# ax-le/nn-fac

Measured on AMD Instinct MI355X. Metric: HALS NMF outer iterations/s (100000x2000 rank-50 row blocks per second), higher is better.
Workload: dtype f32; 1 GPU; NMF hals beta=2, 100000x2000 rank 50 per GPU (configs[1] of BASELINE.json), deterministic (alpha=inf, delta=0.01, maxiter=100); rows_total=100000, cols=2000, rank=50, rows_per_rank=100000, parallelism=single GPU, cost_evaluation=streaming kernel (nnf_frob_resid_f32)

## Files before the change

### nn_fac_amd/csrc/k_hals.hip

```cpp
#include "k_hals_common.h"
#include <cstdlib>

__global__ void nnf_hals_prep_kernel(const float* __restrict__ UtU, int64_t ldg, int r, int RP, float* __restrict__ Gp,
                                     float* __restrict__ dinv, float* __restrict__ Gs, unsigned* counter, double* status) {
    const int RS = 32 * ((RP + 31) / 32);
    const int a = blockIdx.x;
    const float da = (a < r) ? UtU[(int64_t)a * ldg + a] : 0.f;
    const float dia = (da != 0.f) ? (float)(1.0 / (double)da) : 0.f;
    int odd = 0;
    for (int b = threadIdx.x; b < RS; b += blockDim.x) {
        const float g = (a < r && b < r) ? UtU[(int64_t)a * ldg + b] : 0.f;
        odd |= (fabsf(g) < __builtin_inff()) ? 0 : 1;
        Gp[a * RS + b] = g;
        if (Gs) Gs[a * RS + b] = g * dia;
    }
    if (Gs) {
        const int row_odd = __syncthreads_or(odd);
        if (threadIdx.x == 0 && RP < RS) Gs[a * RS + RS - 1] = row_odd ? __builtin_nanf("") : 0.f;
    }
    if (blockIdx.x != 0) return;
    for (int k = threadIdx.x; k < RP; k += blockDim.x) {
        const float d = (k < r) ? UtU[(int64_t)k * ldg + k] : 0.f;
        dinv[2 * k] = (d != 0.f) ? (float)(1.0 / (double)d) : 0.f;
        dinv[2 * k + 1] = (d != 0.f) ? 1.f : 0.f;
    }
    {
        int dead = 0;
        for (int i = threadIdx.x; i < r; i += blockDim.x) dead |= (UtU[(int64_t)i * ldg + i] == 0.f) ? 1 : 0;
        const int any_dead = __syncthreads_or(dead);
        if (threadIdx.x == 0) dinv[2 * RP] = any_dead ? 0.f : 1.f;
    }
    if (threadIdx.x == 0) {
        *counter = 0u;
        if (status) hals_status_defaults(status);
    }
}

template <int MODE, bool GCOL, bool BIG = GCOL>
__global__ __launch_bounds__(128) void nnf_hals_generic_kernel(const float* __restrict__ UtM, int64_t ldm,
                                                               const float* __restrict__ Gp, const float* __restrict__ dinv,
                                                               int RP, float* __restrict__ V, int64_t ldv, int r,
                                                               int64_t ncols, int max_sweeps, double delta, float sp,
                                                               unsigned flags, hals_sync sy, double* __restrict__ status,
                                                               double* __restrict__ sweep_partials, int sweep0,
                                                               float* __restrict__ snapshots, int64_t snap_stride, int snap_first) {
    constexpr int LPC = (BIG && !GCOL) ? 4 : 1;
    constexpr int CW = 128 / LPC;
    extern __shared__ __attribute__((aligned(16))) char smem[];
    float* vl = reinterpret_cast<float*>(smem);
    double* red = reinterpret_cast<double*>(smem + (GCOL ? (size_t)0 : (size_t)r * CW * 4) + 16);
    __shared__ unsigned lds_flag;
    const int nblocks = gridDim.x;
    const int q = threadIdx.x % LPC;
    const int64_t gcolumn = (int64_t)blockIdx.x * CW + threadIdx.x / LPC;
    const bool rowsync = (flags & (NNF_HALS_NORMALIZE | NNF_HALS_NONZERO)) != 0;
    const bool active = gcolumn < ncols;
    const bool owner = active && q == 0;
    unsigned epoch = 0;
    double eps0 = 0.0, eps = 1.0;
    int done = 0, err = 0;
    bool ok = true;
    if (MODE == 0 && sweep0 > 0 && !hals_take_over(status, sweep0, delta, eps0, eps)) return;
    const int64_t col0 = active ? gcolumn : 0;
    float* mycol = GCOL ? V + col0 : vl + threadIdx.x / LPC;
    const int64_t cs = GCOL ? ldv : CW;
    if constexpr (!GCOL) {
        for (int k = q; k < r; k += LPC) mycol[k * CW] = active ? V[(int64_t)k * ldv + col0] : 0.f;
        if constexpr (LPC > 1) __builtin_amdgcn_fence(__ATOMIC_SEQ_CST, "wavefront");
    }
    for (int s = 1; s <= max_sweeps && ok; ++s) {
        double nd = 0.0;
        for (int k = 0; k < r; ++k) {
            const float di = dinv[2 * k];
            if (di != 0.f) {
                float dot = 0.f;
                if constexpr (BIG) {
                    const float* gk = Gp + (size_t)k * RP;
                    float d[8] = {0.f, 0.f, 0.f, 0.f, 0.f, 0.f, 0.f, 0.f};
                    int i = q;
                    for (; i + 7 * LPC < r; i += 8 * LPC) {
                        float gv[8], vv[8];
#pragma unroll
                        for (int u = 0; u < 8; ++u) { gv[u] = gk[i + u * LPC]; vv[u] = mycol[(int64_t)(i + u * LPC) * cs]; }
#pragma unroll
                        for (int u = 0; u < 8; ++u) d[u] = fmaf(gv[u], vv[u], d[u]);
                    }
                    for (int u = 0; i < r; i += LPC, ++u) d[u & 7] = fmaf(gk[i], mycol[(int64_t)i * cs], d[u & 7]);
                    dot = ((d[0] + d[1]) + (d[2] + d[3])) + ((d[4] + d[5]) + (d[6] + d[7]));
                    if constexpr (LPC > 1) {
                        dot += __shfl_xor(dot, 1, 64);
                        dot += __shfl_xor(dot, 2, 64);
                    }
                } else
                for (int i = 0; i < r; ++i) dot = fmaf(Gp[k * RP + i], mycol[i * cs], dot);
                const float vk = mycol[k * cs];
                const float x = (UtM[(int64_t)k * ldm + col0] - dot - sp) * di;
                float step = !(x < -vk) ? x : -vk;
                if (!active) step = 0.f;
                if constexpr (LPC > 1) {
                    __builtin_amdgcn_fence(__ATOMIC_SEQ_CST, "wavefront");
                    if (q == 0) mycol[k * cs] = vk + step;
                    __builtin_amdgcn_fence(__ATOMIC_SEQ_CST, "wavefront");
                    if (q == 0) nd += (double)step * (double)step;
                } else {
                    if (!GCOL || active) mycol[k * cs] = vk + step;
                    nd += (double)step * (double)step;
                }
            } else if (flags & NNF_HALS_NONZERO) {
                err = 2;
            }
            if (rowsync) {
                const float vk = mycol[k * cs];
                double vmax = 0.0;
                if (flags & NNF_HALS_NONZERO) {
                    for (int i = q; i < r; i += LPC) vmax = hals_nanmax(vmax, (double)mycol[i * cs]);
                    if constexpr (LPC > 1) {
                        vmax = hals_nanmax(vmax, __shfl_xor(vmax, 1, 64));
                        vmax = hals_nanmax(vmax, __shfl_xor(vmax, 2, 64));
                    }
                }
                double mine[3] = {owner ? (double)vk * (double)vk : 0.0, (owner && vk != 0.f) ? 1.0 : 0.0,
                                  active ? vmax : -1.0e300};
                double tot[3];
                const double b0 = nnf_block_sum_f64(mine[0], red);
                const double b1 = nnf_block_sum_f64(mine[1], red);
                double bm = mine[2];
                for (int o = 32; o > 0; o >>= 1) bm = hals_nanmax(bm, __shfl_down(bm, o, 64));
                if ((threadIdx.x & 63) == 0) red[threadIdx.x >> 6] = bm;
                __syncthreads();
                bm = hals_nanmax(red[0], red[1]);
                __syncthreads();
                double pub[3] = {b0, b1, bm};
                if (threadIdx.x != 0) { pub[0] = 0; pub[1] = 0; }
                ok = grid_exchange<3>(sy, ++epoch, nblocks, pub, tot, red, &lds_flag);
                if (!ok) break;
                if ((flags & NNF_HALS_NONZERO) && di != 0.f && tot[1] == 0.0 && owner)
                    mycol[k * cs] = (float)(1e-16 * tot[2]);
                if constexpr (LPC > 1) __builtin_amdgcn_fence(__ATOMIC_SEQ_CST, "wavefront");
                if (flags & NNF_HALS_NORMALIZE) {
                    double nsq = tot[0];
                    if ((flags & NNF_HALS_NONZERO) && di != 0.f && tot[1] == 0.0) {
                        const double f = 1e-16 * tot[2];
                        nsq = f * f * (double)ncols;
                    }
                    if (owner) {
                        if (nsq != 0.0) mycol[k * cs] = (float)((double)mycol[k * cs] / sqrt(nsq));
                        else mycol[k * cs] = (float)(1.0 / sqrt((double)ncols));
                    }
                    if constexpr (LPC > 1) __builtin_amdgcn_fence(__ATOMIC_SEQ_CST, "wavefront");
                }
            }
        }
        if (!ok) break;
        done = s;
        const double bs = nnf_block_sum_f64(nd, red);
        if (MODE == 1) {
            if (threadIdx.x == 0) sweep_partials[(size_t)(s - 1) * nblocks + blockIdx.x] = bs;
            if (snapshots != nullptr && s > snap_first && active) {
                float* sn = snapshots + (int64_t)(s - 1 - snap_first) * snap_stride + col0;
                for (int k = q; k < r; k += LPC) sn[(int64_t)k * ncols] = mycol[k * cs];
            }
        } else {
            double mine[1] = {bs}, tot[1];
            ok = grid_exchange<1>(sy, ++epoch, nblocks, mine, tot, red, &lds_flag);
            if (!ok) break;
            if (!hals_note_sum(tot[0], s, sweep0, delta, eps0, eps, done)) break;
        }
    }
    if (!GCOL && active)
        for (int k = q; k < r; k += LPC) V[(int64_t)k * ldv + col0] = mycol[k * CW];
    if (blockIdx.x == 0 && threadIdx.x == 0 && status) {
        hals_status_finish(status, MODE == 0 && max_sweeps >= 1, sweep0, done, eps, eps0, !ok);
        if (ok && err) status[NNF_HALS_ST_ERR] = (double)err;
    }
}

__global__ void nnf_hals_hadamard_kernel(const float* __restrict__ A, const float* __restrict__ B, int64_t ld, int r,
                                        float* __restrict__ out) {
    const int e = blockIdx.x * 256 + threadIdx.x;
    if (e < r * r) out[e] = A[(int64_t)(e / r) * ld + (e % r)] * B[(int64_t)(e / r) * ld + (e % r)];
}

__global__ __launch_bounds__(256) void nnf_hals_sum_sweeps_kernel(const double* __restrict__ partials, int nblocks,
                                                                  double* __restrict__ out) {
    __shared__ double red[4];
    const double* p = partials + (size_t)blockIdx.x * nblocks;
    double s = 0.0;
    for (int b = threadIdx.x; b < nblocks; b += 256) s += p[b];
    const double t = nnf_block_sum_f64(s, red);
    if (threadIdx.x == 0) out[blockIdx.x] = t;
}

struct hals_request {
    int mode;
    const float* UtM; int64_t ldm;
    const float* UtU; const float* UtU2; int64_t ldg;
    float* V; int64_t ldv;
    const float* Vsrc; int64_t ldvs;
    int r; int64_t ncols;
    int nsweeps, sweep0;
    double delta; float sparsity; unsigned flags;
    double* status; double* nodelta;
    float* snapshots; int64_t snap_stride; int snap_first;
    const float* resid_in; float* resid_out;
    hals_shape shape(char force) const {
        return {mode, r, ncols, ldm, ldv, ldvs, nsweeps, sweep0, flags, UtU2 != nullptr, Vsrc != V, snapshots != nullptr, force};
    }
};

static char hals_force() {
    const char* fenv = getenv("NNF_HALS_FORCE");
    return fenv ? fenv[0] : 0;
}

typedef decltype(&nnf_hals_generic_kernel<0, false>) hals_generic_fn;
static hals_generic_fn generic_kernel(int mode, hals_layout l) {
    static const hals_generic_fn k[2][3] = {
        {nnf_hals_generic_kernel<0, false, false>, nnf_hals_generic_kernel<0, false, true>, nnf_hals_generic_kernel<0, true, true>},
        {nnf_hals_generic_kernel<1, false, false>, nnf_hals_generic_kernel<1, false, true>, nnf_hals_generic_kernel<1, true, true>}};
    return k[mode][l - HL_GENERIC_LDS];
}
static int generic_per_cu(int mode, hals_layout l, int r, size_t lds, int cap) {
    static int cached[2][3][HALS_GENERIC_LDS_MAX / 128 + 1];
    static size_t lds_set[2][3];
    const hals_generic_fn k = generic_kernel(mode, l);
    int& c = cached[mode][l - HL_GENERIC_LDS][l == HL_GENERIC_GCOL ? 0 : r];
    if (c == 0) {
        if (l != HL_GENERIC_GCOL && lds > lds_set[mode][l - HL_GENERIC_LDS]) {
            (void)hipFuncSetAttribute(reinterpret_cast<const void*>(k), hipFuncAttributeMaxDynamicSharedMemorySize, (int)lds);
            lds_set[mode][l - HL_GENERIC_LDS] = lds;
        }
        int nb = 0;
        c = hals_per_cu(hipOccupancyMaxActiveBlocksPerMultiprocessor(&nb, k, 128, lds), nb, cap) + 1;
    }
    return c - 1;
}
static const hals_occupancy hals_device_occupancy = {nnf_hals_wave_per_cu, nnf_hals_quad_per_cu, nnf_hals_fast_per_cu,
                                                     nnf_hals_mfma_per_cu, generic_per_cu};

static int hals_entry(nnf_ctx* ctx, hals_request q, hipStream_t st) {
    if (!ctx || !q.UtM || !q.UtU || !q.V || q.r < 1 || q.ncols < 1 || q.ldm < q.ncols || q.ldv < q.ncols || q.ldg < q.r || q.nsweeps < 0)
        return NNF_ERR_ARG;
    if (q.mode == 0 && !q.status) return NNF_ERR_ARG;
    if (q.mode == 1 && !q.nodelta && q.nsweeps > 0) return NNF_ERR_ARG;
    if (q.nsweeps > NNF_HALS_MAX_SWEEPS) return NNF_ERR_UNSUPPORTED;
    if (q.flags & ~(NNF_HALS_SPARSITY | NNF_HALS_NORMALIZE | NNF_HALS_NONZERO)) return NNF_ERR_ARG;
    if (q.Vsrc == nullptr || q.Vsrc == q.V) { q.Vsrc = q.V; q.ldvs = q.ldv; }
    const hals_shape shape = q.shape(hals_force());
    const hals_plan p = hals_make_plan(ctx->num_cus, hals_device_occupancy, shape);
    if (getenv("NNF_HALS_DEBUG")) hals_report(stderr, shape, p);
    if (p.err != NNF_OK) return p.err;

    const bool sweeps = q.nsweeps > 0;
    const int RS = 32 * ((p.RP + 31) / 32);
    nnf_ws_cursor cur(ctx);
    float* Gm = p.mfma_floats ? (float*)cur.take(p.mfma_floats * 4) : nullptr;
    float* Gp = (float*)cur.take(p.gram_floats * 4);
    float* dinv = Gp ? Gp + (size_t)p.RP * RS : nullptr;
    unsigned* counter = (unsigned*)cur.take(256);
    double* slots = (double*)cur.take((size_t)2 * NNF_HALS_MAX_BLOCKS * 4 * 8);
    double* sslots = (q.mode == 0) ? (double*)ctx->xch : slots;
    if (q.mode == 0 && (size_t)(q.nsweeps + 2) * NNF_HALS_MAX_BLOCKS * 16 > ctx->xch_bytes) return NNF_ERR_WORKSPACE;
    const int pslots = p.nblocks > NNF_HALS_MAX_BLOCKS ? p.nblocks : NNF_HALS_MAX_BLOCKS;
    double* partials = q.mode == 1 ? (double*)cur.take((size_t)(sweeps ? q.nsweeps : 1) * pslots * 8) : nullptr;
    float* Gh = p.hadamard ? (float*)cur.take((size_t)q.r * q.r * 4) : nullptr;
    float* snap = p.snap_floats && sweeps ? (float*)cur.take(p.snap_floats * 4) : nullptr;
    if ((p.mfma_floats && !Gm) || !Gp || !counter || !slots || (q.mode == 1 && !partials) || (p.hadamard && !Gh) ||
        (p.snap_floats && sweeps && !snap))
        return NNF_ERR_WORKSPACE;

    if (p.hadamard) {
        hipLaunchKernelGGL(nnf_hals_hadamard_kernel, dim3((q.r * q.r + 255) / 256), dim3(256), 0, st, q.UtU, q.UtU2, q.ldg, q.r, Gh);
        NNF_CHECK_LAUNCH();
        q.UtU = Gh, q.ldg = q.r, q.UtU2 = nullptr;
    }
    const bool native = p.layout == HL_WAVE || p.layout == HL_QUAD;
    auto copy_start_values = [&]() {
        const hipError_t e = hipMemcpy2DAsync(q.V, (size_t)q.ldv * 4, q.Vsrc, (size_t)q.ldvs * 4, (size_t)q.ncols * 4, (size_t)q.r,
                                              hipMemcpyDeviceToDevice, st);
        q.Vsrc = q.V, q.ldvs = q.ldv;
        return e == hipSuccess ? NNF_OK : NNF_ERR_LAUNCH;
    };
    if (p.copy && !native && copy_start_values() != NNF_OK) return NNF_ERR_LAUNCH;
    double* const status0 = (q.mode == 0 && q.sweep0 == 0) ? q.status : nullptr;
    int rc = NNF_OK;
    if (p.prep) {
        if (p.layout == HL_WAVE) rc = nnf_hals_wave_prep(q.UtU, q.UtU2, q.ldg, q.r, Gp, counter, q.status, st);
        else if (p.layout == HL_QUAD) rc = nnf_hals_quad_prep(q.UtU, q.UtU2, q.ldg, q.r, Gp, counter, status0, st);
        else {
            hipLaunchKernelGGL(nnf_hals_prep_kernel, dim3(p.RP), dim3(128), 0, st, q.UtU, q.ldg, q.r, p.RP, Gp, dinv,
                               p.gs ? Gp + hals_gs_off(p.RP) : (float*)nullptr, counter, status0);
            NNF_CHECK_LAUNCH();
        }
        if (rc != NNF_OK) return rc;
    }
    if (p.copy && native && copy_start_values() != NNF_OK) return NNF_ERR_LAUNCH;
    if (!sweeps) return NNF_OK;

    ctx->hals_epoch = (ctx->hals_epoch + 1u) & HALS_EPOCH_MASK;
    if (ctx->hals_epoch == 0u) {
        if (hipMemsetAsync(ctx->xch, 0, ctx->xch_bytes, st) != hipSuccess) return NNF_ERR_LAUNCH;
        ctx->hals_epoch = 1u;
    }
    const hals_sync sy{counter, slots, sslots, ctx->hals_epoch};
    const float sp = (q.flags & NNF_HALS_SPARSITY) ? q.sparsity : 0.f;
    hals_args a{q.UtM, q.ldm, Gp, dinv, p.gs ? Gp + hals_gs_off(p.RP) : nullptr, q.V, q.ldv, q.r, q.ncols, q.nsweeps,
                q.delta, sp, q.mode, sy, q.status, partials, q.snapshots, q.snap_stride, q.sweep0, q.Vsrc, q.ldvs};
    a.snap_first = q.snap_first, a.resid_in = q.resid_in, a.resid_out = q.resid_out;
    const bool probed = p.layout < HL_GENERIC_LDS;
    if (probed) nnf_probe(ctx, NNF_PROBE_HALS, 0, st);
    switch (p.layout) {
        case HL_WAVE:
            a.Gp = q.UtU, a.Gs = q.UtU2, a.dinv = nullptr;
            rc = nnf_hals_wave_launch(p.cpw, p.nw, a, q.ldg, snap, p.nblocks, st);
            break;
        case HL_QUAD: rc = nnf_hals_quad_launch(p.ch, a, Gp, p.nblocks, st); break;
        case HL_MFMA: rc = nnf_hals_mfma_launch(p.RP, q.UtU, q.ldg, Gm, a, p.nblocks, st); break;
        case HL_LANE_RES:
        case HL_LANE_STREAM: rc = nnf_hals_fast_launch(p.RP, p.layout == HL_LANE_RES, a, p.nblocks, st); break;
        default:
            hipLaunchKernelGGL(generic_kernel(q.mode, p.layout), dim3(p.nblocks), dim3(128), p.lds, st, q.UtM, q.ldm, Gp, dinv, RS, q.V,
                               q.ldv, q.r, q.ncols, q.nsweeps, q.delta, sp, q.flags, sy, q.status, partials, q.sweep0, q.snapshots,
                               q.snap_stride, q.snap_first);
            if (hipGetLastError() != hipSuccess) rc = NNF_ERR_LAUNCH;
    }
    if (rc != NNF_OK) return rc;
    if (probed) nnf_probe(ctx, NNF_PROBE_HALS, 1, st);
    if (q.mode == 1) {
        hipLaunchKernelGGL(nnf_hals_sum_sweeps_kernel, dim3(q.nsweeps), dim3(256), 0, st, partials, p.nblocks, q.nodelta);
        NNF_CHECK_LAUNCH();
    }
    return NNF_OK;
}

extern "C" int nnf_hals_solve_f32(nnf_ctx* ctx, const float* UtM, int64_t ldm, const float* UtU, int64_t ldg, float* V,
                                  int64_t ldv, int r, int64_t ncols, int max_sweeps, double delta, float sparsity,
                                  unsigned flags, double* status_f64, void* stream) {
    return hals_entry(ctx, {0, UtM, ldm, UtU, nullptr, ldg, V, ldv, nullptr, 0, r, ncols, max_sweeps, 0, delta, sparsity, flags, status_f64},
                      (hipStream_t)stream);
}

extern "C" int nnf_hals_sweeps_f32(nnf_ctx* ctx, const float* UtM, int64_t ldm, const float* UtU, int64_t ldg, float* V,
                                   int64_t ldv, int r, int64_t ncols, int nsweeps, float sparsity, unsigned flags,
                                   double* nodelta_f64, float* snapshots, int64_t snap_stride, void* stream) {
    return nnf_hals_sweeps_ex_f32(ctx, UtM, ldm, UtU, ldg, V, ldv, r, ncols, nsweeps, 0, sparsity, flags, nodelta_f64, snapshots,
                                  snap_stride, 0, nullptr, nullptr, stream);
}

extern "C" int nnf_hals_sweeps_ex_f32(nnf_ctx* ctx, const float* UtM, int64_t ldm, const float* UtU, int64_t ldg, float* V,
                                      int64_t ldv, int r, int64_t ncols, int nsweeps, int sweeps_done, float sparsity,
                                      unsigned flags, double* nodelta_f64, float* snapshots, int64_t snap_stride, int snap_first,
                                      const float* resid_in, float* resid_out, void* stream) {
    if (sweeps_done < 0 || snap_first < 0 || (snapshots && snap_first >= nsweeps && nsweeps > 0)) return NNF_ERR_ARG;
    if (snapshots && ((flags & (NNF_HALS_NORMALIZE | NNF_HALS_NONZERO)) || snap_stride < (int64_t)r * ncols)) return NNF_ERR_ARG;
    return hals_entry(ctx, {1, UtM, ldm, UtU, nullptr, ldg, V, ldv, nullptr, 0, r, ncols, nsweeps, sweeps_done, 0.0, sparsity, flags, nullptr,
                            nodelta_f64, snapshots, snap_stride, snap_first, resid_in, resid_out}, (hipStream_t)stream);
}

extern "C" int nnf_hals_resid_floats(nnf_ctx* ctx, int r, int64_t ncols, int64_t* floats_out) {
    if (!ctx || r < 1 || ncols < 1 || !floats_out) return NNF_ERR_ARG;
    const hals_shape blind = {1, r, ncols, ncols, ncols, ncols, 1, 0, 0u, false, false, false, hals_force()};
    const hals_plan p = hals_make_plan(ctx->num_cus, hals_device_occupancy, blind);
    *floats_out = (p.err == NNF_OK && p.layout == HL_MFMA) ? (int64_t)nnf_hals_mfma_resid_floats(p.RP, ncols) : 0;
    return NNF_OK;
}

extern "C" int nnf_hals_solve_continue_f32(nnf_ctx* ctx, const float* UtM, int64_t ldm, const float* UtU, int64_t ldg,
                                           float* V, int64_t ldv, int r, int64_t ncols, int sweeps_done, int max_sweeps,
                                           double delta, float sparsity, unsigned flags, double* status_f64, void* stream) {
    if (sweeps_done < 1 || max_sweeps < 1) return NNF_ERR_ARG;
    return hals_entry(ctx, {0, UtM, ldm, UtU, nullptr, ldg, V, ldv, nullptr, 0, r, ncols, max_sweeps, sweeps_done, delta, sparsity, flags,
                            status_f64}, (hipStream_t)stream);
}

__global__ __launch_bounds__(256) void nnf_hals_stop_restore_kernel(const double* __restrict__ sums, int nsweeps, int head,
                                                                   int budget, double delta, float* __restrict__ V, int64_t ldv,
                                                                   int r, int64_t ncols, const float* __restrict__ snapshots,
                                                                   int64_t snap_stride, double* __restrict__ status) {
    __shared__ int s_stop;
    if (threadIdx.x == 0) {
        int stop = -1;
        const double eps0 = sums[0];
        for (int s = 0; s < nsweeps; ++s)
            if (!hals_goes_on(sums[s], delta, eps0) || s + 1 >= budget) { stop = s; break; }
        s_stop = stop;
        if (blockIdx.x == 0) {
            status[NNF_HALS_ST_EPS0] = eps0;
            if (stop < 0) {
                status[NNF_HALS_ST_EPS] = sums[nsweeps - 1];
                status[NNF_HALS_ST_CNT] = (double)(nsweeps + 1);
                status[NNF_HALS_ST_ERR] = 4.0;
            } else {
                status[NNF_HALS_ST_EPS] = sums[stop];
                status[NNF_HALS_ST_CNT] = (double)(stop + 2);
                status[NNF_HALS_ST_ERR] = (stop < head) ? 3.0 : 0.0;
            }
        }
    }
    __syncthreads();
    const int stop = s_stop;
    if (stop < head || stop >= nsweeps - 1) return;
    const float* src = snapshots + (int64_t)(stop - head) * snap_stride;
    const int64_t total = (int64_t)r * ncols;
    for (int64_t e = (int64_t)blockIdx.x * 256 + threadIdx.x; e < total; e += (int64_t)gridDim.x * 256) {
        const int64_t k = e / ncols, j = e - k * ncols;
        V[k * ldv + j] = src[k * ncols + j];
    }
}

extern "C" int nnf_hals_resident_columns(nnf_ctx* ctx, int r, int64_t* columns_out) {
    if (!ctx || r < 1 || !columns_out) return NNF_ERR_ARG;
    const int64_t columns = hals_resident_columns(ctx->num_cus, hals_device_occupancy, r);
    if (columns < 1) return NNF_ERR_LAUNCH;
    *columns_out = columns;
    return NNF_OK;
}

extern "C" int nnf_hals_stop_restore_f32(nnf_ctx* ctx, const double* sums_f64, int nsweeps, int head, int budget, double delta,
                                         float* V, int64_t ldv, int r, int64_t ncols, const float* snapshots,
                                         int64_t snap_stride, double* status_f64, void* stream) {
    if (!ctx || !sums_f64 || !V || !status_f64 || nsweeps < 1 || head < 0 || head >= nsweeps || budget < 1 || r < 1 ||
        ncols < 1 || ldv < ncols)
        return NNF_ERR_ARG;
    if (nsweeps - head > 1 && (!snapshots || snap_stride < (int64_t)r * ncols)) return NNF_ERR_ARG;
    int64_t grid = nnf_cdiv((int64_t)r * ncols, 256 * 8);
    if (grid > 2048) grid = 2048;
    if (grid < 1) grid = 1;
    hipLaunchKernelGGL(nnf_hals_stop_restore_kernel, dim3((int)grid), dim3(256), 0, (hipStream_t)stream, sums_f64, nsweeps, head,
                       budget, delta, V, ldv, r, ncols, snapshots, snap_stride, status_f64);
    NNF_CHECK_LAUNCH();
    return NNF_OK;
}

extern "C" int nnf_hals_solve_cross_f32(nnf_ctx* ctx, const float* UtM, int64_t ldm, const float* UtU_a, const float* UtU_b,
                                        int64_t ldg, const float* V_in, int64_t ldvi, float* V_out, int64_t ldvo, int r,
                                        int64_t ncols, int max_sweeps, double delta, float sparsity, unsigned flags,
                                        double* status_f64, void* stream) {
    if (!V_in || ldvi < ncols) return NNF_ERR_ARG;
    if (max_sweeps > NNF_HALS_MAX_SWEEPS) return NNF_ERR_UNSUPPORTED;
    return hals_entry(ctx, {0, UtM, ldm, UtU_a, UtU_b, ldg, V_out, ldvo, V_in, ldvi, r, ncols, max_sweeps, 0, delta, sparsity, flags,
                            status_f64}, (hipStream_t)stream);
}

__global__ __launch_bounds__(256) void nnf_hals_row_update_kernel(const float* __restrict__ UtM, int64_t ldm, const float* __restrict__ UtU,
                                                                  int64_t ldg, float* __restrict__ V, int64_t ldv, int r, int64_t ncols,
                                                                  int k, float sp, double* __restrict__ partial) {
    __shared__ double red[4];
    const float d = UtU[(int64_t)k * ldg + k];
    const float di = (d != 0.f) ? (float)(1.0 / (double)d) : 0.f;
    double nd = 0.0, nv = 0.0;
    for (int64_t col = (int64_t)blockIdx.x * 256 + threadIdx.x; col < ncols; col += (int64_t)gridDim.x * 256) {
        float vk = V[(int64_t)k * ldv + col];
        if (di != 0.f) {
            float dot = 0.f;
            for (int i = 0; i < r; ++i) dot = fmaf(UtU[(int64_t)k * ldg + i], V[(int64_t)i * ldv + col], dot);
            const float x = (UtM[(int64_t)k * ldm + col] - dot - sp) * di;
            const float step = !(x < -vk) ? x : -vk;
            vk += step;
            V[(int64_t)k * ldv + col] = vk;
            nd += (double)step * (double)step;
        }
        nv += (double)vk * (double)vk;
    }
    const double bd = nnf_block_sum_f64(nd, red), bv = nnf_block_sum_f64(nv, red);
    if (threadIdx.x == 0) {
        partial[blockIdx.x] = bd;
        partial[gridDim.x + blockIdx.x] = bv;
    }
}
__global__ __launch_bounds__(256) void nnf_hals_row_sums_kernel(const double* __restrict__ partial, int nwg, double* __restrict__ out2) {
    __shared__ double red[4];
    for (int q = 0; q < 2; ++q) {
        double s = 0.0;
        for (int e = threadIdx.x; e < nwg; e += 256) s += partial[(size_t)q * nwg + e];
        const double t = nnf_block_sum_f64(s, red);
        if (threadIdx.x == 0) out2[q] = t;
    }
}
__global__ __launch_bounds__(256) void nnf_hals_row_scale_kernel(float* __restrict__ V, int64_t ncols, const double* __restrict__ normsq,
                                                                 double fill) {
    const double nsq = normsq[0];
    for (int64_t col = (int64_t)blockIdx.x * 256 + threadIdx.x; col < ncols; col += (int64_t)gridDim.x * 256)
        V[col] = (nsq != 0.0) ? (float)((double)V[col] / sqrt(nsq)) : (float)fill;
}
extern "C" int nnf_hals_row_update_f32(nnf_ctx* ctx, const float* UtM, int64_t ldm, const float* UtU, int64_t ldg, float* V, int64_t ldv,
                                       int r, int64_t ncols, int k, float sparsity, unsigned flags, double* out2_f64, void* stream) {
    if (!ctx || !UtM || !UtU || !V || !out2_f64 || r < 1 || ncols < 1 || k < 0 || k >= r || ldm < ncols || ldv < ncols || ldg < r)
        return NNF_ERR_ARG;
    if (flags & ~NNF_HALS_SPARSITY) return NNF_ERR_ARG;
    hipStream_t st = (hipStream_t)stream;
    int64_t grid = nnf_cdiv(ncols, 256);
    if (grid > 2048) grid = 2048;
    nnf_ws_cursor cur(ctx);
    double* partial = (double*)cur.take((size_t)2 * grid * 8);
    if (!partial) return NNF_ERR_WORKSPACE;
    hipLaunchKernelGGL(nnf_hals_row_update_kernel, dim3((int)grid), dim3(256), 0, st, UtM, ldm, UtU, ldg, V, ldv, r, ncols, k,
                       (flags & NNF_HALS_SPARSITY) ? sparsity : 0.f, partial);
    NNF_CHECK_LAUNCH();
    hipLaunchKernelGGL(nnf_hals_row_sums_kernel, dim3(1), dim3(256), 0, st, partial, (int)grid, out2_f64);
    NNF_CHECK_LAUNCH();
    return NNF_OK;
}
extern "C" int nnf_hals_row_scale_f32(nnf_ctx* ctx, float* V, int64_t ldv, int64_t ncols, int k, const double* normsq_f64,
                                      int64_t ncols_total, void* stream) {
    if (!ctx || !V || !normsq_f64 || ncols < 1 || k < 0 || ldv < ncols || ncols_total < ncols) return NNF_ERR_ARG;
    int64_t grid = nnf_cdiv(ncols, 256);
    if (grid > 2048) grid = 2048;
    hipLaunchKernelGGL(nnf_hals_row_scale_kernel, dim3((int)grid), dim3(256), 0, (hipStream_t)stream, V + (int64_t)k * ldv, ncols,
                       normsq_f64, 1.0 / sqrt((double)ncols_total));
    NNF_CHECK_LAUNCH();
    return NNF_OK;
}
```

### nn_fac_amd/csrc/k_hals_common.h

```cpp
#pragma once
#include "nnf_internal.h"
#include "k_hals_plan.h"

typedef __amdgpu_buffer_rsrc_t rsrc_t;
typedef float f32x2 __attribute__((ext_vector_type(2)));

#define HALS_SPIN_LIMIT (1u << 22)


struct hals_sync {
    unsigned* counter;
    double* slots;
    double* sslots;
    unsigned epoch;
};

__device__ __forceinline__ double hals_nanmax(double x, double y) { return (y > x || y != y) ? y : x; }

template <int NV>
__device__ __forceinline__ bool grid_exchange(const hals_sync& sy, unsigned epoch, int nblocks, const double (&mine)[NV],
                                              double (&out)[NV], double* red, unsigned* lds_flag) {
    double* slot = sy.slots + ((size_t)(epoch & 1) * nblocks + blockIdx.x) * 4;
    if (threadIdx.x == 0) {
#pragma unroll
        for (int i = 0; i < NV; ++i)
            __hip_atomic_store(reinterpret_cast<unsigned long long*>(slot + i), __builtin_bit_cast(unsigned long long, mine[i]),
                               __ATOMIC_RELAXED, __HIP_MEMORY_SCOPE_AGENT);
        asm volatile("s_waitcnt vmcnt(0)" ::: "memory");
        __hip_atomic_fetch_add(sy.counter, 1u, __ATOMIC_RELAXED, __HIP_MEMORY_SCOPE_AGENT);
        const unsigned target = epoch * (unsigned)nblocks;
        unsigned spins = 0, ok = 1;
        while (__hip_atomic_load(sy.counter, __ATOMIC_RELAXED, __HIP_MEMORY_SCOPE_AGENT) < target) {
            __builtin_amdgcn_s_sleep(2);
            if (++spins > HALS_SPIN_LIMIT) { ok = 0; break; }
        }
        *lds_flag = ok;
    }
    __syncthreads();
    const bool ok = (*lds_flag != 0);
    double s[NV];
#pragma unroll
    for (int i = 0; i < NV; ++i) s[i] = (i == 2) ? -1.0e300 : 0.0;
    const double* base = sy.slots + (size_t)(epoch & 1) * nblocks * 4;
    for (int b = threadIdx.x; b < nblocks; b += blockDim.x) {
#pragma unroll
        for (int i = 0; i < NV; ++i) {
            const double x = __builtin_bit_cast(
                double, __hip_atomic_load(reinterpret_cast<const unsigned long long*>(base + (size_t)b * 4 + i),
                                          __ATOMIC_RELAXED, __HIP_MEMORY_SCOPE_AGENT));
            if (i == 2) s[i] = hals_nanmax(s[i], x); else s[i] += x;
        }
    }
    const int w = threadIdx.x >> 6, nw = (blockDim.x + 63) >> 6;
#pragma unroll
    for (int i = 0; i < NV; ++i) {
        double v = s[i];
#pragma unroll
        for (int o = 32; o > 0; o >>= 1) {
            const double y = __shfl_down(v, o, 64);
            if (i == 2) v = hals_nanmax(v, y); else v += y;
        }
        if ((threadIdx.x & 63) == 0) red[w * NV + i] = v;
    }
    __syncthreads();
#pragma unroll
    for (int i = 0; i < NV; ++i) {
        double v = red[i];
        for (int k = 1; k < nw; ++k) {
            const double y = red[k * NV + i];
            if (i == 2) v = hals_nanmax(v, y); else v += y;
        }
        out[i] = v;
    }
    __syncthreads();
    return ok;
}


constexpr unsigned HALS_TAG_STRIDE = 1024u;
constexpr unsigned HALS_EPOCH_MASK = 0xffffffffu / HALS_TAG_STRIDE;
static_assert(NNF_HALS_MAX_SWEEPS + 2 <= HALS_TAG_STRIDE, "every sweep row of a launch has a tag of its own");
static_assert((HALS_EPOCH_MASK & (HALS_EPOCH_MASK + 1u)) == 0u, "the host wraps the epoch with this mask");
typedef unsigned long long hals_word;
__device__ __forceinline__ unsigned hals_tag(const hals_sync& sy, int s) { return sy.epoch * HALS_TAG_STRIDE + (unsigned)s; }
__device__ __forceinline__ const hals_word* hals_row(const hals_sync& sy, int s, int nblocks) {
    return reinterpret_cast<const hals_word*>(sy.sslots) + (size_t)s * nblocks * 2;
}
__device__ __forceinline__ double hals_granule_value(hals_word g0, hals_word g1) {
    return __builtin_bit_cast(double, (g1 << 32) | (g0 & 0xffffffffull));
}
__device__ __forceinline__ bool hals_granule_wait(const hals_word* row, int b, unsigned tag, hals_word& g0, hals_word& g1) {
    unsigned spins = 0;
    while (!((unsigned)(g0 >> 32) == tag && (unsigned)(g1 >> 32) == tag)) {
        if (spins > 0) __builtin_amdgcn_s_sleep(1);
        if (++spins > HALS_SPIN_LIMIT) return false;
        g0 = __hip_atomic_load(row + 2 * (size_t)b, __ATOMIC_RELAXED, __HIP_MEMORY_SCOPE_AGENT);
        g1 = __hip_atomic_load(row + 2 * (size_t)b + 1, __ATOMIC_RELAXED, __HIP_MEMORY_SCOPE_AGENT);
    }
    return true;
}
__device__ __forceinline__ void hals_publish(const hals_sync& sy, int s, int nblocks, double mine, bool me = threadIdx.x == 0) {
    if (me) {
        const hals_word bits = __builtin_bit_cast(hals_word, mine);
        const hals_word tag = (hals_word)hals_tag(sy, s) << 32;
        hals_word* g = reinterpret_cast<hals_word*>(sy.sslots) + ((size_t)s * nblocks + blockIdx.x) * 2;
        __hip_atomic_store(g, tag | (bits & 0xffffffffull), __ATOMIC_RELAXED, __HIP_MEMORY_SCOPE_AGENT);
        __hip_atomic_store(g + 1, tag | (bits >> 32), __ATOMIC_RELAXED, __HIP_MEMORY_SCOPE_AGENT);
    }
}
constexpr int HALS_PF = 2;
struct hals_prefetch {
    hals_word g0[HALS_PF], g1[HALS_PF];
    int s;
};
__device__ __forceinline__ void hals_collect_issue(const hals_sync& sy, int s, int nblocks, hals_prefetch& pf) {
    const hals_word* base = hals_row(sy, s, nblocks);
    pf.s = s;
#pragma unroll
    for (int i = 0; i < HALS_PF; ++i) {
        const int b = threadIdx.x + i * blockDim.x;
        pf.g0[i] = pf.g1[i] = 0ull;
        if (b < nblocks) {
            pf.g0[i] = __hip_atomic_load(base + 2 * (size_t)b, __ATOMIC_RELAXED, __HIP_MEMORY_SCOPE_AGENT);
            pf.g1[i] = __hip_atomic_load(base + 2 * (size_t)b + 1, __ATOMIC_RELAXED, __HIP_MEMORY_SCOPE_AGENT);
        }
    }
}
__device__ __forceinline__ bool hals_collect(const hals_sync& sy, int s, int nblocks, double& total, double* red,
                                             unsigned* lds_flag, const hals_prefetch* pf = nullptr) {
    if (threadIdx.x == 0) *lds_flag = 1u;
    __syncthreads();
    const unsigned tag = hals_tag(sy, s);
    const hals_word* base = hals_row(sy, s, nblocks);
    double v = 0.0;
    int i = 0;
    for (int b = threadIdx.x; b < nblocks; b += blockDim.x, ++i) {
        hals_word g0 = 0ull, g1 = 0ull;
        if (pf != nullptr && pf->s == s) {
#pragma unroll
            for (int u = 0; u < HALS_PF; ++u)
                if (u == i) { g0 = pf->g0[u]; g1 = pf->g1[u]; }
        }
        if (!hals_granule_wait(base, b, tag, g0, g1)) *lds_flag = 0u;
        v += hals_granule_value(g0, g1);
    }
    v = nnf_wave_sum_f64(v);
    const int w = threadIdx.x >> 6, nw = (blockDim.x + 63) >> 6;
    if ((threadIdx.x & 63) == 0) red[w] = v;
    __syncthreads();
    const bool ok = (*lds_flag != 0);
    double t = red[0];
    for (int k = 1; k < nw; ++k) t += red[k];
    total = t;
    __syncthreads();
    return ok;
}

#ifndef HALS_DBG
#define HALS_DBG 0
#endif
#ifndef HALS_LATE_ISSUE
#define HALS_LATE_ISSUE 1
#endif
#ifndef HALS_MID_AT
#define HALS_MID_AT(R) ((R) - 1)
#endif
struct hals_mid_none {
    __device__ __forceinline__ void operator()() const {}
};
struct hals_mid_issue {
    unsigned long long a0, a1;
    hals_prefetch& pf;
    __device__ __forceinline__ void operator()() const {
        static_assert(HALS_PF == 2, "two granule pairs per thread");
        asm volatile("global_load_dwordx2 %0, %4, off sc1\n\tglobal_load_dwordx2 %1, %4, off offset:8 sc1\n\t"
                     "global_load_dwordx2 %2, %5, off sc1\n\tglobal_load_dwordx2 %3, %5, off offset:8 sc1"
                     : "=&v"(pf.g0[0]), "=&v"(pf.g1[0]), "=&v"(pf.g0[1]), "=&v"(pf.g1[1])
                     : "v"(a0), "v"(a1));
    }
};
__device__ __forceinline__ void hals_mid_wait(hals_prefetch& pf) {
    asm volatile("s_waitcnt vmcnt(0)" : "+v"(pf.g0[0]), "+v"(pf.g1[0]), "+v"(pf.g0[1]), "+v"(pf.g1[1]));
}

__device__ __forceinline__ bool hals_collect1(const hals_sync& sy, int s, int nblocks, double& total, double* red_p,
                                              unsigned* lds_flag, const hals_prefetch& pf) {
    const unsigned tag = hals_tag(sy, s);
    const hals_word* base = hals_row(sy, s, nblocks);
    double v = 0.0;
    int i = 0;
    for (int b = threadIdx.x; b < nblocks; b += blockDim.x, ++i) {
        hals_word g0 = 0ull, g1 = 0ull;
        if (pf.s == s) {
#pragma unroll
            for (int u = 0; u < HALS_PF; ++u)
                if (u == i) { g0 = pf.g0[u]; g1 = pf.g1[u]; }
        }
        unsigned spins = 0;
        while (!((unsigned)(g0 >> 32) == tag && (unsigned)(g1 >> 32) == tag)) {
            if (spins > 0) __builtin_amdgcn_s_sleep(1);
            if (++spins > HALS_SPIN_LIMIT) { *lds_flag = 0u; break; }
            g0 = __hip_atomic_load(base + 2 * (size_t)b, __ATOMIC_RELAXED, __HIP_MEMORY_SCOPE_AGENT);
            g1 = __hip_atomic_load(base + 2 * (size_t)b + 1, __ATOMIC_RELAXED, __HIP_MEMORY_SCOPE_AGENT);
        }
        v += hals_granule_value(g0, g1);
    }
    v = nnf_wave_sum_f64(v);
    const int w = threadIdx.x >> 6, nw = (blockDim.x + 63) >> 6;
    if ((threadIdx.x & 63) == 0) red_p[w] = v;
    __syncthreads();
    double t = red_p[0];
    for (int k = 1; k < nw; ++k) t += red_p[k];
    total = t;
    return *lds_flag != 0u;
}

__device__ __forceinline__ bool hals_collect_wave(const hals_sync& sy, int s, int nblocks, double& total,
                                                  const hals_prefetch* pf = nullptr) {
    const unsigned tag = hals_tag(sy, s);
    const hals_word* base = hals_row(sy, s, nblocks);
    double v = 0.0;
    bool late = false;
    int i = 0;
    for (int b = threadIdx.x; b < nblocks; b += 64, ++i) {
        hals_word g0 = 0ull, g1 = 0ull;
        if (pf != nullptr && pf->s == s) {
#pragma unroll
            for (int u = 0; u < HALS_PF; ++u)
                if (u == i) { g0 = pf->g0[u]; g1 = pf->g1[u]; }
        }
        if (!hals_granule_wait(base, b, tag, g0, g1)) late = true;
        v += hals_granule_value(g0, g1);
    }
    total = nnf_wave_sum_f64(v);
    return __ballot(late) == 0ull;
}

template <int NT>
__device__ __forceinline__ bool hals_sum_collect1(const hals_sync& sy, double nd, double& bs, int c, int nblocks, double& total,
                                                  double* red_bs, double* red_tot, unsigned* lds_flag,
                                                  const hals_prefetch& pf) {
    static_assert(NT == 256 && HALS_PF == 2, "two granule pairs per thread cover nblocks <= 512");
    const unsigned tag = hals_tag(sy, c);
    const hals_word* base = hals_row(sy, c, nblocks);
    hals_word g0[HALS_PF], g1[HALS_PF];
    bool want[HALS_PF], need = false;
#pragma unroll
    for (int i = 0; i < HALS_PF; ++i) {
        want[i] = (int)threadIdx.x + NT * i < nblocks;
        g0[i] = (pf.s == c) ? pf.g0[i] : 0ull;
        g1[i] = (pf.s == c) ? pf.g1[i] : 0ull;
        need = need || (want[i] && !((unsigned)(g0[i] >> 32) == tag && (unsigned)(g1[i] >> 32) == tag));
    }
    if (!(HALS_DBG & 1) && __builtin_expect(__ballot(need) != 0ull, 0)) {
#pragma unroll 1
        for (int i = 0; i < HALS_PF; ++i) {
            const int b = (int)threadIdx.x + NT * i;
            hals_word a0 = i == 0 ? g0[0] : g0[HALS_PF - 1], a1 = i == 0 ? g1[0] : g1[HALS_PF - 1];
            if (b < nblocks && !hals_granule_wait(base, b, tag, a0, a1)) *lds_flag = 0u;
            if (i == 0) { g0[0] = a0; g1[0] = a1; } else { g0[HALS_PF - 1] = a0; g1[HALS_PF - 1] = a1; }
        }
    }
    double v = 0.0;
#pragma unroll
    for (int i = 0; i < HALS_PF; ++i)
        v += want[i] ? hals_granule_value(g0[i], g1[i]) : 0.0;
    v = nnf_wave_sum_f64(v);
    nd = nnf_wave_sum_f64(nd);
    constexpr int nw = NT / 64;
    const int w = threadIdx.x >> 6;
    if ((threadIdx.x & 63) == 0) { red_bs[w] = nd; red_tot[w] = v; }
    __syncthreads();
    double t = red_tot[0], b2 = red_bs[0];
#pragma unroll
    for (int k = 1; k < nw; ++k) { t += red_tot[k]; b2 += red_bs[k]; }
    total = t;
    bs = b2;
    return *lds_flag != 0u;
}
template <int NT>
__device__ __forceinline__ double hals_block_sum1(double v, double* red_p) {
    v = nnf_wave_sum_f64(v);
    constexpr int nw = NT / 64;
    const int w = threadIdx.x >> 6;
    if ((threadIdx.x & 63) == 0) red_p[w] = v;
    __syncthreads();
    double t = red_p[0];
#pragma unroll
    for (int k = 1; k < nw; ++k) t += red_p[k];
    return t;
}

struct hals_args {
    const float* UtM; int64_t ldm;
    const float* Gp;
    const float* dinv;
    const float* Gs;
    float* V; int64_t ldv;
    int r; int64_t ncols;
    int max_sweeps; double delta; float sp;
    int mode;
    hals_sync sy;
    double* status;
    double* sweep_partials;
    float* snapshots;
    int64_t snap_stride;
    int sweep0;
    const float* Vsrc;
    int64_t ldvs;
    const float* Mimg;
    const float* Mlt;
    int rp;
    const float* resid_in;
    float* resid_out;
    int snap_first;
};

__device__ __forceinline__ bool hals_goes_on(double eps, double delta, double eps0) { return eps >= delta * eps0; }
__device__ __forceinline__ bool hals_note_sum(double tot, int c, int sweep0, double delta, double& eps0, double& eps, int& done) {
    if (c == 1 && sweep0 == 0) eps0 = tot;
    eps = tot;
    done = c;
    return hals_goes_on(eps, delta, eps0);
}
__device__ __forceinline__ bool hals_take_over(const double* status, int sweep0, double delta, double& eps0, double& eps) {
    const double pe = status[NNF_HALS_ST_EPS], pe0 = status[NNF_HALS_ST_EPS0];
    if ((int)status[NNF_HALS_ST_CNT] - 1 != sweep0 || !(pe >= delta * pe0) || status[NNF_HALS_ST_ERR] != 0.0) return false;
    eps0 = pe0;
    eps = pe;
    return true;
}

__device__ __forceinline__ void hals_status_defaults(double* st, double err = 0.0) {
    st[NNF_HALS_ST_EPS] = 1.0;
    st[NNF_HALS_ST_CNT] = 1.0;
    st[NNF_HALS_ST_EPS0] = 0.0;
    st[NNF_HALS_ST_ERR] = err;
}
__device__ __forceinline__ void hals_status_finish(double* st, bool ran, int sweep0, int done, double eps, double eps0, bool timed_out) {
    if (ran) {
        st[NNF_HALS_ST_EPS] = eps;
        st[NNF_HALS_ST_CNT] = (double)(sweep0 + done + 1);
        st[NNF_HALS_ST_EPS0] = eps0;
    }
    if (timed_out) st[NNF_HALS_ST_ERR] = 1.0;
}

static inline int hals_per_cu(hipError_t e, int nb, int cap) {
    if (e != hipSuccess || nb < 1) return 0;
    const int b = nb >= 3 ? nb - 1 : nb;
    return cap > 0 && b > cap ? cap : b;
}


int nnf_hals_fast_per_cu(int RP, bool resident);
int nnf_hals_fast_launch(int RP, bool resident, const hals_args& a, int nblocks, hipStream_t);

int nnf_hals_wave_per_cu(int r, int cpw, int nw);
int nnf_hals_wave_prep(const float* UtU, const float* UtU2, int64_t ldg, int r, float* Gw, unsigned* counter, double* status,
                       hipStream_t);
int nnf_hals_wave_launch(int cpw, int nw, const hals_args& a, int64_t ldg, float* snap, int nblocks, hipStream_t);

int nnf_hals_mfma_per_cu(int RP);
int nnf_hals_mfma_launch(int RP, const float* UtU, int64_t ldg, float* gram, hals_args a, int nblocks, hipStream_t);

int nnf_hals_quad_per_cu(int ch);
int nnf_hals_quad_prep(const float* UtU, const float* UtU2, int64_t ldg, int r, float* Gq, unsigned* counter, double* status,
                       hipStream_t);
int nnf_hals_quad_launch(int ch, hals_args a, float* Gq, int nblocks, hipStream_t);
```

### nn_fac_amd/csrc/k_hals_fast.hip

```cpp
#include "k_hals_common.h"
#include "k_parts.h"

#ifndef HALS_PART
#error "compile with -DHALS_PART=<part>"
#endif
#define NNF_PART HALS_PART

NNF_BUILD_FLAGS(NNF_CAT(k_hals_fast, HALS_PART), "HALS_LATE_ISSUE=" NNF_STR(HALS_LATE_ISSUE) " HALS_MID_AT(R)=" NNF_STR(HALS_MID_AT(R)) " HALS_DBG=" NNF_STR(HALS_DBG))

typedef float f32x16 __attribute__((ext_vector_type(16)));
typedef float f32x8 __attribute__((ext_vector_type(8)));

#define NNF_SLOAD2(d0, d1, base, off) \
    asm volatile("s_load_dwordx16 %0, %2, %3\n\ts_load_dwordx16 %1, %2, %4" : "=&s"(d0), "=&s"(d1) : "s"(base), "i"((off) * 4), "i"((off) * 4 + 64))
#define NNF_SLOAD2D(d0, d1, dd, base, off, doff) \
    asm volatile("s_load_dwordx16 %0, %3, %4\n\ts_load_dwordx16 %1, %3, %5\n\ts_load_dword %2, %3, %6" \
                 : "=&s"(d0), "=&s"(d1), "=&s"(dd) : "s"(base), "i"((off) * 4), "i"((off) * 4 + 64), "i"((doff) * 4))
#define NNF_SWAIT2(d0, d1) asm volatile("s_waitcnt lgkmcnt(0)" : "+s"(d0), "+s"(d1))
#define NNF_SWAIT3(d0, d1, dd) asm volatile("s_waitcnt lgkmcnt(0)" : "+s"(d0), "+s"(d1), "+s"(dd))

template <int W>
struct sgbuf {
    f32x16 a, b;
    f32x8 q;
    f32x4 r;
};
template <int W, bool TIED>
__device__ __forceinline__ void sg_issue(sgbuf<W>& d, uint64_t base, int off) {
    constexpr int N16 = W / 16, N8 = (W % 16) / 8, N4 = (W % 8) / 4;
    static_assert(W % 4 == 0 && N16 <= 2, "piece decomposition");
    if constexpr (TIED) {
        if constexpr (N16 >= 1) asm volatile("s_load_dwordx16 %0, %1, %2" : "+s"(d.a) : "s"(base), "i"(off * 4));
        if constexpr (N16 >= 2) asm volatile("s_load_dwordx16 %0, %1, %2" : "+s"(d.b) : "s"(base), "i"(off * 4 + 64));
        if constexpr (N8 == 1) asm volatile("s_load_dwordx8 %0, %1, %2" : "+s"(d.q) : "s"(base), "i"(off * 4 + 64 * N16));
        if constexpr (N4 == 1) asm volatile("s_load_dwordx4 %0, %1, %2" : "+s"(d.r) : "s"(base), "i"(off * 4 + 64 * N16 + 32 * N8));
    } else {
        if constexpr (N16 >= 1) asm volatile("s_load_dwordx16 %0, %1, %2" : "=s"(d.a) : "s"(base), "i"(off * 4));
        if constexpr (N16 >= 2) asm volatile("s_load_dwordx16 %0, %1, %2" : "=s"(d.b) : "s"(base), "i"(off * 4 + 64));
        if constexpr (N8 == 1) asm volatile("s_load_dwordx8 %0, %1, %2" : "=s"(d.q) : "s"(base), "i"(off * 4 + 64 * N16));
        if constexpr (N4 == 1) asm volatile("s_load_dwordx4 %0, %1, %2" : "=s"(d.r) : "s"(base), "i"(off * 4 + 64 * N16 + 32 * N8));
    }
}
template <int W>
__device__ __forceinline__ void sg_arrived(sgbuf<W>& d) {
    constexpr int N16 = W / 16, N8 = (W % 16) / 8, N4 = (W % 8) / 4;
    if constexpr (N16 >= 1) asm volatile("" : "+s"(d.a));
    if constexpr (N16 >= 2) asm volatile("" : "+s"(d.b));
    if constexpr (N8 == 1) asm volatile("" : "+s"(d.q));
    if constexpr (N4 == 1) asm volatile("" : "+s"(d.r));
}
template <int W>
__device__ __forceinline__ f32x2 sg_pair(const sgbuf<W>& d, int p) {
    constexpr int N16 = W / 16, N8 = (W % 16) / 8;
    const int j = 2 * p;
    if (N16 >= 1 && j < 16) return f32x2{d.a[j], d.a[j + 1]};
    if (N16 >= 2 && j < 32) return f32x2{d.b[j - 16], d.b[j - 15]};
    const int j2 = j - 16 * N16;
    if (N8 == 1 && j2 < 8) return f32x2{d.q[j2], d.q[j2 + 1]};
    const int j3 = j2 - 8 * N8;
    return f32x2{d.r[j3], d.r[j3 + 1]};
}

template <int R, bool GUARD, class MID>
__device__ __forceinline__ float hals_sweep_column_xy(f32x2 (&v2)[R / 2], const float (&b)[R], const float* __restrict__ Gs,
                                                      const float* __restrict__ nzp, const MID& mid) {
    constexpr int RS = 64, P = R / 2, YW = 24, XW = (R - YW + 3) & ~3, XP = XW / 2;
    static_assert(YW == 24, "the Y issue statement below is written for x16 + x8");
    static_assert(R > 32 && R <= 64 && R % 2 == 0 && XW + YW <= RS && XW >= 8, "row split");
    const uint64_t base = (uint64_t)Gs, nzb = (uint64_t)nzp;
    sgbuf<XW> X;
    sgbuf<YW> Y[2];
    f32x2 dv[2];
    float nd = 0.f;
    sg_issue<XW, false>(X, base, 0);
    sg_issue<YW, false>(Y[0], base, XW);
    if constexpr (GUARD) asm volatile("s_load_dwordx2 %0, %1, %2" : "=s"(dv[0]) : "s"(nzb), "i"(0));
#pragma unroll
    for (int k = 0; k < R; ++k) {
        const int cur = k & 1, nxt = cur ^ 1;
        if (k == HALS_MID_AT(R)) mid();
        if constexpr (GUARD) asm volatile("s_waitcnt lgkmcnt(0)" : "+s"(dv[cur]));
        else asm volatile("s_waitcnt lgkmcnt(0)" ::: "memory");
        sg_arrived<XW>(X);
        sg_arrived<YW>(Y[cur]);
        if (k + 1 < R) {
            if constexpr (GUARD)
                asm volatile("s_load_dwordx16 %0, %3, %4\n\ts_load_dwordx8 %1, %3, %5\n\ts_load_dwordx2 %2, %6, %7"
                             : "=&s"(Y[nxt].a), "=&s"(Y[nxt].q), "=&s"(dv[nxt])
                             : "s"(base), "i"(((k + 1) * RS + XW) * 4), "i"(((k + 1) * RS + XW + 16) * 4), "s"(nzb),
                               "i"(8 * (k + 1)));
            else
                asm volatile("s_load_dwordx16 %0, %2, %3\n\ts_load_dwordx8 %1, %2, %4"
                             : "=&s"(Y[nxt].a), "=&s"(Y[nxt].q)
                             : "s"(base), "i"(((k + 1) * RS + XW) * 4), "i"(((k + 1) * RS + XW + 16) * 4));
        }
        f32x2 a0 = {0.f, 0.f}, a1 = {0.f, 0.f};
#pragma unroll
        for (int p = 0; p < XP; ++p) {
            const f32x2 g = sg_pair<XW>(X, p);
            if (p & 1) a1 = __builtin_elementwise_fma(g, v2[p], a1);
            else a0 = __builtin_elementwise_fma(g, v2[p], a0);
        }
        asm volatile("" : "+v"(a0), "+v"(a1));
        if (k + 1 < R) sg_issue<XW, true>(X, base, (k + 1) * RS);
#pragma unroll
        for (int p = XP; p < P; ++p) {
            const f32x2 g = sg_pair<YW>(Y[cur], p - XP);
            if (p & 1) a1 = __builtin_elementwise_fma(g, v2[p], a1);
            else a0 = __builtin_elementwise_fma(g, v2[p], a0);
        }
        const f32x2 a = a0 + a1;
        const float vk = v2[k / 2][k & 1];
        const float x = b[k] - (a[0] + a[1]);
        float dl;
        if constexpr (GUARD) {
            const float sel = !(x < -vk) ? x : -vk;
            asm("v_mul_legacy_f32 %0, %1, %2" : "=v"(dl) : "s"(dv[cur][1]), "v"(sel));
        } else {
            asm("v_max_f32 %0, %1, -%2" : "=v"(dl) : "v"(x), "v"(vk));
        }
        v2[k / 2][k & 1] = vk + dl;
        nd = fmaf(dl, dl, nd);
        asm volatile("" : "+v"(nd));
    }
    return nd;
}

template <int R, bool KEEPB, class MID>
__device__ __forceinline__ float hals_sweep_column(f32x2 (&v2)[R / 2], const float (&b)[KEEPB ? R : 1], rsrc_t rb, int voff,
                                                   int ldm4, const float* __restrict__ Gp, float sp, const MID& mid) {
    constexpr int NBLK = (R + 31) / 32, RS = 32 * NBLK, P = R / 2, DOFF = R * RS;
    const uint64_t base = (uint64_t)Gp;
    f32x16 buf[2][2];
    float dv[2];
    float nd = 0.f;
    constexpr int BPF = 8;
    float bring[KEEPB ? 1 : BPF];
    if constexpr (!KEEPB) {
#pragma unroll
        for (int i = 0; i < BPF; ++i)
            bring[i] = __builtin_bit_cast(float, __builtin_amdgcn_raw_buffer_load_b32(rb, voff, i * ldm4, 0));
    }
    NNF_SLOAD2D(buf[0][0], buf[0][1], dv[0], base, 0, DOFF);
#pragma unroll
    for (int k = 0; k < R; ++k) {
        if (k == HALS_MID_AT(R)) mid();
        f32x2 a0 = {0.f, 0.f}, a1 = {0.f, 0.f}, a2 = {0.f, 0.f}, a3 = {0.f, 0.f};
        float di = 0.f;
#pragma unroll
        for (int blk = 0; blk < NBLK; ++blk) {
            const int jb = k * NBLK + blk, cur = jb & 1, nxt = cur ^ 1;
            if (blk == 0) {
                NNF_SWAIT3(buf[cur][0], buf[cur][1], dv[k & 1]);
                di = dv[k & 1];
            } else {
                NNF_SWAIT2(buf[cur][0], buf[cur][1]);
            }
            if (blk + 1 < NBLK) {
                NNF_SLOAD2(buf[nxt][0], buf[nxt][1], base, k * RS + 32 * (blk + 1));
            } else if (k + 1 < R) {
                NNF_SLOAD2D(buf[nxt][0], buf[nxt][1], dv[(k + 1) & 1], base, (k + 1) * RS, DOFF + 2 * (k + 1));
            }
#pragma unroll
            for (int j = 0; j < 8; j += 2) {
                if (16 * blk + j < P)
                    a0 = __builtin_elementwise_fma(f32x2{buf[cur][0][2 * j], buf[cur][0][2 * j + 1]}, v2[16 * blk + j], a0);
                if (16 * blk + 8 + j < P)
                    a1 = __builtin_elementwise_fma(f32x2{buf[cur][1][2 * j], buf[cur][1][2 * j + 1]}, v2[16 * blk + 8 + j], a1);
                if (16 * blk + j + 1 < P)
                    a2 = __builtin_elementwise_fma(f32x2{buf[cur][0][2 * j + 2], buf[cur][0][2 * j + 3]}, v2[16 * blk + j + 1], a2);
                if (16 * blk + 8 + j + 1 < P)
                    a3 = __builtin_elementwise_fma(f32x2{buf[cur][1][2 * j + 2], buf[cur][1][2 * j + 3]}, v2[16 * blk + 8 + j + 1], a3);
            }
        }
        const f32x2 a = (a0 + a1) + (a2 + a3);
        const float dot = a[0] + a[1];
        float bk;
        if constexpr (KEEPB) {
            bk = b[k];
        } else {
            bk = bring[k % BPF];
            if (k + BPF < R)
                bring[k % BPF] = __builtin_bit_cast(float, __builtin_amdgcn_raw_buffer_load_b32(rb, voff, (k + BPF) * ldm4, 0));
        }
        const float vk = v2[k / 2][k & 1];
        const bool skip = __builtin_bit_cast(unsigned, di) == 0u;
        const float res = KEEPB ? (bk - dot) : (bk - dot - sp);
        const float x = (skip ? 0.f : res) * di;
        const float t = vk + x;
        const bool keep = !(t <= 0.f) | skip;
        const float vn = keep ? t : 0.f;
        const float step = keep ? x : -vk;
        v2[k / 2][k & 1] = vn;
        nd = fmaf(step, step, nd);
        asm volatile("" : "+v"(nd));
    }
    return nd;
}

template <int RP, bool RES>
__global__ __launch_bounds__(256, (RP > 104 ? 1 : 2)) void nnf_hals_kernel(hals_args a) {
    constexpr bool KEEPB = (RP <= 104);
    constexpr bool XY = (RP > 32 && RP <= 52);
    const bool all_live = XY && (a.dinv[2 * RP] != 0.f);
    __shared__ double red[4 * 3];
    __shared__ double red2[2][2][4];
    __shared__ unsigned lds_flag;
    if (threadIdx.x == 0) lds_flag = 1u;
    const int nblocks = gridDim.x;
    const int64_t gthreads = (int64_t)nblocks * 256;
    const int64_t gtid = (int64_t)blockIdx.x * 256 + threadIdx.x;
    const rsrc_t rv = __builtin_amdgcn_make_buffer_rsrc(a.V, 0, (int)(((int64_t)(a.r - 1) * a.ldv + a.ncols) * 4), 0x00020000);
    const rsrc_t rb = __builtin_amdgcn_make_buffer_rsrc(const_cast<float*>(a.UtM), 0,
                                                        (int)(((int64_t)(a.r - 1) * a.ldm + a.ncols) * 4), 0x00020000);
    const int ldv4 = (int)(a.ldv * 4), ldm4 = (int)(a.ldm * 4);
    const rsrc_t rvs = __builtin_amdgcn_make_buffer_rsrc(const_cast<float*>(a.Vsrc), 0,
                                                         (int)(((int64_t)(a.r - 1) * a.ldvs + a.ncols) * 4), 0x00020000);
    const int ldvs4 = (int)(a.ldvs * 4);
    f32x2 v2[RP / 2];
    float b[KEEPB ? RP : 1];
    bool plain = false;
    auto sweep = [&](int voff, const auto& mid) -> float {
        if constexpr (XY) {
            return plain ? hals_sweep_column_xy<RP, false>(v2, b, a.Gs, a.dinv, mid) : hals_sweep_column_xy<RP, true>(v2, b, a.Gs, a.dinv, mid);
        } else {
            return hals_sweep_column<RP, KEEPB>(v2, b, rb, voff, ldm4, a.Gp, a.sp, mid);
        }
    };
    auto load_col = [&](int voff) {
#pragma unroll
        for (int k = 0; k < RP; ++k) {
            v2[k / 2][k & 1] = RES ? __builtin_bit_cast(float, __builtin_amdgcn_raw_buffer_load_b32(rvs, voff, k * ldvs4, 0))
                                   : __builtin_bit_cast(float, __builtin_amdgcn_raw_buffer_load_b32(rv, voff, k * ldv4, 0));
            if constexpr (KEEPB) {
                b[k] = __builtin_bit_cast(float, __builtin_amdgcn_raw_buffer_load_b32(rb, voff, k * ldm4, 0)) - a.sp;
                if constexpr (XY) b[k] *= a.dinv[2 * k];
            }
        }
    };
    auto store_col = [&](int voff) {
#pragma unroll
        for (int k = 0; k < RP; ++k) {
            const float val = v2[k / 2][k & 1];
            __builtin_amdgcn_raw_buffer_store_b32(__builtin_bit_cast(unsigned, val), rv, voff, k * ldv4, 0);
        }
    };
    const int voff0 = gtid < a.ncols ? (int)(gtid * 4) : (int)0x7ffffff0;
    if constexpr (RES) load_col(voff0);
    if constexpr (RES && XY) {
        static_assert(!XY || RP < 64, "the scaled Gram's rows have a spare last float");
        float c = a.Gs[(threadIdx.x & 63) < RP ? (threadIdx.x & 63) * 64 + 63 : 63];
#pragma unroll
        for (int k = 0; k < RP; ++k) {
            c = fmaf(v2[k / 2][k & 1], 0.f, c);
            c = fmaf(b[k], 0.f, c);
            asm volatile("" : "+v"(c));
        }
        plain = all_live && __ballot(!(c == 0.f)) == 0ull;
    }
    constexpr bool BACKUP = RES && RP <= 64;
    constexpr bool SPEC = BACKUP;
    f32x2 vb[BACKUP ? RP / 2 : 1];

    double eps0 = 0.0, eps = 1.0;
    int done = 0;
    bool ok = true, stopped = false;
    if (a.mode == 0 && a.sweep0 > 0 && !hals_take_over(a.status, a.sweep0, a.delta, eps0, eps)) return;
    hals_prefetch pf;
    pf.s = 0;
    for (int s = 1; s <= a.max_sweeps; ++s) {
        double nd = 0.0;
        if constexpr (BACKUP) {
            if (a.mode == 0) {
#pragma unroll
                for (int k = 0; k < RP / 2; ++k) vb[k] = v2[k];
            }
        }
        if constexpr (RES) {
            float f;
            if constexpr (SPEC && (RP > 52 || !HALS_LATE_ISSUE)) {
                if (a.mode == 0 && s >= 2) hals_collect_issue(a.sy, s - 1, nblocks, pf);
                f = sweep(voff0, hals_mid_none{});
            } else if constexpr (SPEC) {
                const bool want = a.mode == 0 && s >= 2;
                const hals_word* row = hals_row(a.sy, want ? s - 1 : 0, nblocks);
                const int b0 = (int)threadIdx.x < nblocks ? (int)threadIdx.x : 0;
                const int b1 = (int)threadIdx.x + 256 < nblocks ? (int)threadIdx.x + 256 : 0;
                pf.s = want ? s - 1 : 0;
                f = sweep(voff0, hals_mid_issue{(unsigned long long)(row + 2 * (size_t)b0), (unsigned long long)(row + 2 * (size_t)b1), pf});
                hals_mid_wait(pf);
            } else {
                f = sweep(voff0, hals_mid_none{});
            }
            nd = gtid < a.ncols ? (double)f : 0.0;
        } else {
            for (int64_t col = gtid; col < a.ncols; col += gthreads) {
                const int voff = (int)(col * 4);
                load_col(voff);
                nd += (double)sweep(voff, hals_mid_none{});
                store_col(voff);
            }
        }
        double bs;
        bool merged = false;
        double tot_m = 0.0;
        if constexpr (RES && SPEC) {
            if (a.mode == 0 && s >= 2 && !(HALS_DBG & 6)) {
                ok = hals_sum_collect1<256>(a.sy, nd, bs, s - 1, nblocks, tot_m, red2[s & 1][0], red2[s & 1][1], &lds_flag, pf);
                merged = true;
            }
        }
        if (!merged) {
            if constexpr (RES) bs = hals_block_sum1<256>(nd, red2[s & 1][0]);
            else bs = nnf_block_sum_f64(nd, red);
        }
        if (a.mode == 1) {
            if (threadIdx.x == 0) a.sweep_partials[(size_t)(s - 1) * nblocks + blockIdx.x] = bs;
            if constexpr (RES) {
                if (a.snapshots != nullptr && gtid < a.ncols && s > a.snap_first) {
                    float* sp_ = a.snapshots + (size_t)(s - 1 - a.snap_first) * a.snap_stride + gtid;
#pragma unroll
                    for (int k = 0; k < RP; ++k)
                        if (k < a.r) sp_[(int64_t)k * a.ncols] = v2[k / 2][k & 1];
                }
            }
            done = s;
            continue;
        }
        if (!(HALS_DBG & 4)) hals_publish(a.sy, s, nblocks, bs);
        const int c = SPEC ? s - 1 : s;
        if (c >= 1 && !(HALS_DBG & 6)) {
            double tot;
            if (merged) tot = tot_m;
            else if constexpr (RES) ok = hals_collect1(a.sy, c, nblocks, tot, red2[s & 1][1], &lds_flag, pf);
            else ok = hals_collect(a.sy, c, nblocks, tot, red, &lds_flag, &pf);
            if (!ok) break;
            if (c == 1 && a.sweep0 == 0) eps0 = tot;
            eps = tot;
            done = c;
            if (!(eps >= a.delta * eps0) && !HALS_DBG) { stopped = true; break; }
        }
    }
    if constexpr (RES) {
        if (a.mode == 0) {
            if constexpr (BACKUP) {
                if (stopped || !ok) {
#pragma unroll
                    for (int k = 0; k < RP / 2; ++k) v2[k] = vb[k];
                }
            }
            if (a.max_sweeps >= 1) store_col(voff0);
        }
    }
    if (a.mode == 1) {
        if constexpr (RES) store_col(voff0);
    } else if (SPEC && ok && !stopped && a.max_sweeps >= 1 && !HALS_DBG) {
        double tot;
        ok = hals_collect(a.sy, a.max_sweeps, nblocks, tot, red, &lds_flag);
        if (ok) {
            if (a.max_sweeps == 1 && a.sweep0 == 0) eps0 = tot;
            eps = tot;
            done = a.max_sweeps;
        }
    }
    if (a.mode == 0 && blockIdx.x == 0 && threadIdx.x == 0)
        hals_status_finish(a.status, a.max_sweeps >= 1, a.sweep0, done, eps, eps0, !ok);
}

template <int RP>
static int fast_per_cu(bool res) {
    static int cached[2] = {-1, -1};
    int& c = cached[res ? 1 : 0];
    if (c < 0) {
        int nb = 0;
        const hipError_t e = res ? hipOccupancyMaxActiveBlocksPerMultiprocessor(&nb, nnf_hals_kernel<RP, true>, 256, 0)
                                 : hipOccupancyMaxActiveBlocksPerMultiprocessor(&nb, nnf_hals_kernel<RP, false>, 256, 0);
        c = hals_per_cu(e, nb, 3);
    }
    return c;
}

template <int RP>
static int fast_launch(bool res, const hals_args& a, int nblocks, hipStream_t st) {
    if (res) hipLaunchKernelGGL((nnf_hals_kernel<RP, true>), dim3(nblocks), dim3(256), 0, st, a);
    else hipLaunchKernelGGL((nnf_hals_kernel<RP, false>), dim3(nblocks), dim3(256), 0, st, a);
    NNF_CHECK_LAUNCH();
    return NNF_OK;
}

#define HALS_TABLE(X)                                                                                            \
    X(0, 8) X(0, 16) X(0, 24) X(0, 32) X(0, 40) X(0, 48)                                                         \
    X(1, 50) X(1, 52) X(1, 56) X(1, 64)                                                                          \
    X(2, 80) X(2, 96)                                                                                            \
    X(3, 100)                                                                                                    \
    X(4, 104)                                                                                                    \
    X(5, 112) X(5, 128)
NNF_PART_DISPATCHER(fast_mine, HALS_TABLE)

int NNF_CAT(nnf_hals_fast_per_cu_part, HALS_PART)(int RP, bool res) {
    return fast_mine(RP, 0, [&](auto rp) { return fast_per_cu<decltype(rp)::value>(res); });
}
int NNF_CAT(nnf_hals_fast_launch_part, HALS_PART)(int RP, bool res, const hals_args& a, int nblocks, hipStream_t st) {
    return fast_mine(RP, NNF_ERR_UNSUPPORTED, [&](auto rp) { return fast_launch<decltype(rp)::value>(res, a, nblocks, st); });
}

#if HALS_PART == 0
#define HALS_DECLARE(p, v)                                      \
    int NNF_PART_FN(nnf_hals_fast_per_cu_part, p)(int, bool);   \
    int NNF_PART_FN(nnf_hals_fast_launch_part, p)(int, bool, const hals_args&, int, hipStream_t);
#define HALS_PER_CU(p, v) case v: return NNF_PART_FN(nnf_hals_fast_per_cu_part, p)(RP, res);
#define HALS_LAUNCH(p, v) case v: return NNF_PART_FN(nnf_hals_fast_launch_part, p)(RP, res, a, nblocks, st);
HALS_TABLE(HALS_DECLARE)
int nnf_hals_fast_per_cu(int RP, bool res) {
    switch (RP) { HALS_TABLE(HALS_PER_CU) default: return 0; }
}
int nnf_hals_fast_launch(int RP, bool res, const hals_args& a, int nblocks, hipStream_t st) {
    switch (RP) { HALS_TABLE(HALS_LAUNCH) default: return NNF_ERR_UNSUPPORTED; }
}
#endif
```

### nn_fac_amd/csrc/k_hals_plan.h

```cpp
#pragma once
#include "k_stream_plan.h"

#define NNF_HALS_MAX_SWEEPS 1000
#define NNF_HALS_MAX_BLOCKS 2048

enum hals_layout { HL_WAVE, HL_QUAD, HL_MFMA, HL_LANE_RES, HL_LANE_STREAM, HL_GENERIC_LDS, HL_GENERIC_BIG, HL_GENERIC_GCOL };
static const char* const hals_layout_name[] = {"wave", "quad", "mfma", "lane-resident", "lane-streaming", "generic-lds",
                                               "generic-lds-big", "generic-gcol"};

struct hals_shape {
    int mode;
    int r; int64_t ncols;
    int64_t ldm, ldv, ldvs;
    int nsweeps, sweep0;
    unsigned flags;
    bool gram2;
    bool own_start;
    bool snapshots;
    char force;
};

struct hals_plan {
    int err = NNF_OK;
    hals_layout layout = HL_LANE_RES;
    int RP = 0, nblocks = 0, per_cu = 0;
    int cpw = 0, nw = 0, ch = 0;
    size_t lds = 0;
    bool hadamard = false, copy = false, prep = true;
    bool gs = false;
    size_t gram_floats = 0, mfma_floats = 0, snap_floats = 0;
};

struct hals_occupancy {
    int (*wave)(int r, int cpw, int nw);
    int (*quad)(int ch);
    int (*lane)(int RP, bool resident);
    int (*mfma)(int RP);
    int (*generic)(int mode, hals_layout layout, int r, size_t lds_bytes, int cap);
};

static inline int pick_rp(int r) {
    const int opts[] = {8, 16, 24, 32, 40, 48, 50, 52, 56, 64, 80, 96, 100, 104, 112, 128};
    for (int o : opts)
        if (r <= o) return o;
    return (r + 7) & ~7;
}

constexpr int WAVE_COMM = 4;
constexpr int WAVE_MAX_NW = 16 - WAVE_COMM;
constexpr int WAVE_SNAP = 16;
constexpr int WAVE_NP = 6;
static inline int wave_ru(int r) { return (r + 7) & ~7; }
static inline int wave_rl(int r) { return r <= 64 ? 1 : 2; }
static inline size_t nnf_hals_wave_gram_floats(int r) { return (size_t)wave_ru(r) * 64 * wave_rl(r) + 128; }
static inline size_t nnf_hals_wave_snap_floats(int r, int64_t ncols) { return (size_t)ncols * WAVE_SNAP * 64 * wave_rl(r); }
static inline int nnf_hals_wave_grid(int64_t ncols, int cpw, int* nw_out) {
    int nw = (int)nnf_cdiv(ncols, 256);
    if (nw < 1) nw = 1;
    if (nw > WAVE_MAX_NW) nw = WAVE_MAX_NW;
    *nw_out = nw;
    const int64_t need = nnf_cdiv(ncols, (int64_t)nw * cpw);
    return need > 64 * WAVE_NP ? 0 : (int)need;
}

static inline size_t nnf_hals_quad_gram_floats(int r) {
    const int ch = (r + 3) / 4, rq = 4 * ch, rs = 4 * ((ch + 3) & ~3);
    return (size_t)rq * rs + rq;
}

struct mfma_shape { int rt, rem, nkb; };
static inline bool mfma_shape_of(int RP, mfma_shape& s) {
    switch (RP) {
        case 48: s = {3, 0, 12}; return true;
        case 50: s = {3, 2, 13}; return true;
        case 52: s = {3, 4, 13}; return true;
        case 64: s = {4, 0, 16}; return true;
        case 80: s = {5, 0, 20}; return true;
        case 96: s = {6, 0, 24}; return true;
        case 100: s = {6, 4, 25}; return true;
        default: return false;
    }
}
static inline bool nnf_hals_mfma_supported(int RP) { mfma_shape s; return mfma_shape_of(RP, s); }
static inline size_t nnf_hals_mfma_gram_floats(int RP) {
    mfma_shape s;
    if (!mfma_shape_of(RP, s)) return 0;
    return (size_t)s.nkb * ((s.rt + 3) / 4) * 256 + (size_t)s.nkb * 32 + 64;
}
static inline size_t nnf_hals_mfma_resid_floats(int RP, int64_t ncols) {
    mfma_shape s;
    if (!mfma_shape_of(RP, s) || ncols < 1) return 0;
    return (size_t)nnf_cdiv(ncols, 256) * 4 * (s.rt * 4 + 1) * 256;
}

constexpr size_t HALS_GENERIC_LDS_MAX = (size_t)150 * 1024;
constexpr size_t HALS_GENERIC_SHM_FIXED = 16 + 3 * 2 * 8 + 64;

static inline int64_t hals_cap(int cus, int per_cu) {
    const int64_t c = (int64_t)per_cu * cus;
    return c < NNF_HALS_MAX_BLOCKS ? c : NNF_HALS_MAX_BLOCKS;
}
static inline bool hals_32bit(int rows, int64_t ld, int64_t ncols) {
    return (((int64_t)(rows - 1) * ld + ncols) * 4) < (int64_t)0x7fff0000;
}

static inline size_t hals_gs_off(int RP) { return ((((size_t)RP * (32 * ((RP + 31) / 32)) + 2 * RP + 1) + 15) & ~(size_t)15); }

static inline hals_plan hals_refuse(hals_plan p, int err) { p.err = err; return p; }

static inline hals_plan hals_make_plan(int cus, const hals_occupancy& occ, const hals_shape& q) {
    hals_plan p;
    const int r = q.r; const int64_t n = q.ncols;
    const bool rowsync = (q.flags & (NNF_HALS_NORMALIZE | NNF_HALS_NONZERO)) != 0;
    const bool generic = r > NNF_MAX_RANK || rowsync;
    const bool sweeps = q.nsweeps > 0;
    const char force = q.force;
    p.RP = pick_rp(r);
    const bool mfma = !generic && sweeps && force != 'l' && force != 'q' && force != 'w' && nnf_hals_mfma_supported(p.RP) &&
                      (force == 'm' || (p.RP >= 64 && n > 32768));
    const bool pin_mfma = force == 'm' && mfma;

    const bool wave_shape = !generic && q.mode == 0 && q.sweep0 == 0;
    if (wave_shape && force != 'l' && force != 'q' && !pin_mfma) {
        for (int cpw = 1; cpw <= 2; ++cpw) {
            int nw = 0;
            const int need = nnf_hals_wave_grid(n, cpw, &nw);
            if (need < 1 || need > NNF_HALS_MAX_BLOCKS) continue;
            const int pc = occ.wave(r, cpw, nw);
            if (pc < 1) break;
            if (need <= (int64_t)pc * cus) {
                p.layout = HL_WAVE, p.cpw = cpw, p.nw = nw, p.nblocks = need, p.per_cu = pc;
                p.prep = !sweeps;
                p.copy = !sweeps && q.own_start;
                p.gram_floats = nnf_hals_wave_gram_floats(r);
                p.snap_floats = nnf_hals_wave_snap_floats(r, n);
                return p;
            }
        }
    }
    if (force == 'w' && wave_shape) return hals_refuse(p, NNF_ERR_UNSUPPORTED);

    auto quad_32bit = [&](int64_t ld) { return (int64_t)(r + 16) * ld * 4 < (int64_t)0x7fff0000; };
    if (!generic && force != 'l' && !pin_mfma && (n <= 32768 || force == 'q') && quad_32bit(q.ldv > q.ldm ? q.ldv : q.ldm)) {
        const int ch = (r + 3) / 4, pc = occ.quad(ch);
        const int64_t need = nnf_cdiv(n, 16);
        if (pc > 0 && need <= hals_cap(cus, pc)) {
            p.layout = HL_QUAD, p.ch = ch, p.nblocks = (int)need, p.per_cu = pc;
            p.copy = q.own_start && (!sweeps || !quad_32bit(q.ldvs));
            p.gram_floats = nnf_hals_quad_gram_floats(r);
            return p;
        }
    }

    const int RS = 32 * ((p.RP + 31) / 32);
    p.gs = !generic && p.RP > 32 && p.RP <= 52;
    p.gram_floats = hals_gs_off(p.RP) + (p.gs ? (size_t)p.RP * RS : 0);
    p.hadamard = q.gram2;
    const int lane_pc = generic ? 0 : occ.lane(p.RP, true);
    const bool lane_fits = lane_pc > 0 && nnf_cdiv(n, 256) <= hals_cap(cus, lane_pc);
    p.copy = q.own_start && !(!generic && sweeps && lane_fits && hals_32bit(p.RP, q.ldvs, n));
    if (!sweeps) {
        p.layout = generic ? HL_GENERIC_LDS : HL_LANE_RES;
        return p;
    }

    if (generic) {
        const bool exchanges = q.mode == 0 || rowsync;
        if (r > NNF_MAX_RANK) {
            p.layout = HL_GENERIC_BIG;
            p.lds = (size_t)r * 32 * 4 + HALS_GENERIC_SHM_FIXED;
            p.per_cu = p.lds <= HALS_GENERIC_LDS_MAX ? occ.generic(q.mode, HL_GENERIC_BIG, r, p.lds, 0) : 0;
            if (p.per_cu < 1 || (exchanges && nnf_cdiv(n, 32) > hals_cap(cus, p.per_cu))) {
                p.layout = HL_GENERIC_GCOL;
                p.lds = HALS_GENERIC_SHM_FIXED;
                p.per_cu = occ.generic(q.mode, HL_GENERIC_GCOL, r, p.lds, 4);
            }
        } else {
            p.layout = HL_GENERIC_LDS;
            p.lds = (size_t)r * 128 * 4 + HALS_GENERIC_SHM_FIXED;
            p.per_cu = occ.generic(q.mode, HL_GENERIC_LDS, r, p.lds, 4);
        }
        if (p.per_cu < 1) return hals_refuse(p, NNF_ERR_LAUNCH);
        const int64_t grid = nnf_cdiv(n, p.layout == HL_GENERIC_BIG ? 32 : 128);
        if (grid > (exchanges ? hals_cap(cus, p.per_cu) : (int64_t)0x7fffffff)) return hals_refuse(p, NNF_ERR_UNSUPPORTED);
        p.nblocks = (int)grid;
        return p;
    }

    if (!hals_32bit(p.RP, q.ldv, n) || !hals_32bit(p.RP, q.ldm, n)) return hals_refuse(p, NNF_ERR_UNSUPPORTED);
    const int64_t need = nnf_cdiv(n, 256);
    if (mfma) {
        const int pc = occ.mfma(p.RP);
        if (pc > 0 && need <= hals_cap(cus, pc)) {
            p.layout = HL_MFMA, p.nblocks = (int)need, p.per_cu = pc;
            p.mfma_floats = nnf_hals_mfma_gram_floats(p.RP);
            return p;
        }
    }
    if (lane_pc < 1) return hals_refuse(p, NNF_ERR_LAUNCH);
    if (lane_fits) {
        p.layout = HL_LANE_RES, p.nblocks = (int)need, p.per_cu = lane_pc;
        return p;
    }
    if (q.snapshots) return hals_refuse(p, NNF_ERR_UNSUPPORTED);
    p.layout = HL_LANE_STREAM, p.per_cu = occ.lane(p.RP, false);
    if (p.per_cu < 1) return hals_refuse(p, NNF_ERR_LAUNCH);
    p.nblocks = (int)hals_cap(cus, p.per_cu);
    return p;
}

static inline void hals_report(FILE* f, const hals_shape& q, const hals_plan& p, const char* more = "") {
    fprintf(f, "[nnf hals] r=%d ncols=%lld mode=%d sweeps=%d sweep0=%d flags=%u -> %s grid=%d per_cu=%d cpw=%d nw=%d ch=%d "
            "RP=%d gs=%d lds=%zu hadamard=%d copy=%d prep=%d err=%d%s\n", q.r, (long long)q.ncols, q.mode, q.nsweeps, q.sweep0,
            q.flags, hals_layout_name[p.layout], p.nblocks, p.per_cu, p.cpw, p.nw, p.ch, p.RP, p.gs, p.lds, p.hadamard, p.copy,
            p.prep, p.err, more);
}

static inline int64_t hals_resident_columns(int cus, const hals_occupancy& occ, int r) {
    if (r > NNF_MAX_RANK) return hals_cap(cus, occ.generic(0, HL_GENERIC_GCOL, r, HALS_GENERIC_SHM_FIXED, 4)) * 128;
    return hals_cap(cus, occ.lane(pick_rp(r), true)) * 256;
}
```

Baseline: 1299 iterations/s.

## Add lane-resident HALS kernel with a dedicated wave for convergence reduction

Adds a new resident HALS kernel for ranks 33–52. Each 576-thread workgroup has eight compute waves that sweep 512 columns, plus one extra wave that does the grid-wide delta reduction and convergence verdict asynchronously. The compute waves go on to the next sweep without waiting for the grid exchange, and restore a saved copy of V if the verdict says to stop. This is meant to hide grid-synchronisation latency behind computation. The right-hand side moves to LDS, and the planner picks this path when the column count needs more lane blocks than there are CUs. The cost is one block per CU, one extra speculative sweep at the end, and extra register copies of V.

New measurement: 1335 iterations/s, median of 6. 1.03x the previous value.

```diff
diff --git a/nn_fac_amd/csrc/k_hals.hip b/nn_fac_amd/csrc/k_hals.hip
--- a/nn_fac_amd/csrc/k_hals.hip
+++ b/nn_fac_amd/csrc/k_hals.hip
@@ -236,7 +236,7 @@
     return c - 1;
 }
 static const hals_occupancy hals_device_occupancy = {nnf_hals_wave_per_cu, nnf_hals_quad_per_cu, nnf_hals_fast_per_cu,
-                                                     nnf_hals_mfma_per_cu, generic_per_cu};
+                                                     nnf_hals_mfma_per_cu, generic_per_cu, nnf_hals_comm_per_cu};
 
 static int hals_entry(nnf_ctx* ctx, hals_request q, hipStream_t st) {
     if (!ctx || !q.UtM || !q.UtU || !q.V || q.r < 1 || q.ncols < 1 || q.ldm < q.ncols || q.ldv < q.ncols || q.ldg < q.r || q.nsweeps < 0)
@@ -317,6 +317,8 @@
         case HL_QUAD: rc = nnf_hals_quad_launch(p.ch, a, Gp, p.nblocks, st); break;
         case HL_MFMA: rc = nnf_hals_mfma_launch(p.RP, q.UtU, q.ldg, Gm, a, p.nblocks, st); break;
         case HL_LANE_RES:
+            if (p.comm) { rc = nnf_hals_comm_launch(p.RP, a, p.nblocks, st); break; }
+            [[fallthrough]];
         case HL_LANE_STREAM: rc = nnf_hals_fast_launch(p.RP, p.layout == HL_LANE_RES, a, p.nblocks, st); break;
         default:
             hipLaunchKernelGGL(generic_kernel(q.mode, p.layout), dim3(p.nblocks), dim3(128), p.lds, st, q.UtM, q.ldm, Gp, dinv, RS, q.V,
diff --git a/nn_fac_amd/csrc/k_hals_comm.hip b/nn_fac_amd/csrc/k_hals_comm.hip
--- /dev/null
+++ b/nn_fac_amd/csrc/k_hals_comm.hip
@@ -0,0 +1,245 @@
+#include "k_hals_common.h"
+#include "k_hals_lane_sweep.h"
+
+constexpr int LC_CW = 8;
+constexpr int LC_COLS = 64 * LC_CW;
+constexpr int LC_THREADS = LC_COLS + 64;
+constexpr int LC_RING = 4;
+constexpr int LC_NP = 8;
+static_assert(LC_COLS == HALS_B_PITCH, "one row of b_lds holds the workgroup's columns");
+
+struct lane_ctl {
+    unsigned tag[LC_RING][LC_CW];
+    unsigned long long ver[LC_RING];
+    unsigned fin;
+};
+static inline size_t lc_lds_bytes(int RP) { return ((size_t)RP + 2) * LC_COLS * 4 + sizeof(lane_ctl); }
+
+#define LC_WG __HIP_MEMORY_SCOPE_WORKGROUP
+
+__device__ __forceinline__ void lc_publish(const hals_sync& sy, int s, int ngran, int gi, double mine) {
+    const hals_word bits = __builtin_bit_cast(hals_word, mine);
+    const hals_word tag = (hals_word)hals_tag(sy, s) << 32;
+    hals_word* g = reinterpret_cast<hals_word*>(sy.sslots) + ((size_t)s * ngran + gi) * 2;
+    __hip_atomic_store(g, tag | (bits & 0xffffffffull), __ATOMIC_RELAXED, __HIP_MEMORY_SCOPE_AGENT);
+    __hip_atomic_store(g + 1, tag | (bits >> 32), __ATOMIC_RELAXED, __HIP_MEMORY_SCOPE_AGENT);
+}
+
+__device__ __forceinline__ bool lc_wait_tags(const lane_ctl* ctl, int c, int lane) {
+    unsigned spins = 0;
+    for (;;) {
+        const unsigned t = __hip_atomic_load(&ctl->tag[c & (LC_RING - 1)][lane & (LC_CW - 1)], __ATOMIC_ACQUIRE, LC_WG);
+        if (__ballot(t != (unsigned)c) == 0ull) return true;
+        if (__hip_atomic_load(&ctl->fin, __ATOMIC_RELAXED, LC_WG) != 0u) return false;
+        __builtin_amdgcn_s_sleep(4);
+        if (++spins > HALS_SPIN_LIMIT) return false;
+    }
+}
+
+__device__ __forceinline__ double lc_sum4x64(double x0, double x1, double x2, double x3) {
+    double v = (x0 + x1) + (x2 + x3);
+    v = nnf_dpp_add_f64<0xB1, 0xf>(v);
+    v = nnf_dpp_add_f64<0x4E, 0xf>(v);
+    v = nnf_dpp_add_f64<0x141, 0xf>(v);
+    v = nnf_dpp_add_f64<0x140, 0xf>(v);
+    return v;
+}
+__device__ __forceinline__ double lc_rows_in_order(double v) {
+    const unsigned long long u = __builtin_bit_cast(unsigned long long, v);
+    double t = 0.0;
+#pragma unroll
+    for (int k = 0; k < 4; ++k) {
+        const unsigned lo = (unsigned)__builtin_amdgcn_readlane((int)(unsigned)u, 16 * k);
+        const unsigned hi = (unsigned)__builtin_amdgcn_readlane((int)(unsigned)(u >> 32), 16 * k);
+        const double w = __builtin_bit_cast(double, ((unsigned long long)hi << 32) | (unsigned long long)lo);
+        t = k == 0 ? w : t + w;
+    }
+    return t;
+}
+
+__device__ __forceinline__ double lc_half_sum(const float* nd_half, int lane) {
+    const f32x4 x = *reinterpret_cast<const f32x4*>(nd_half + 4 * lane);
+    return lc_rows_in_order(lc_sum4x64((double)x[0], (double)x[1], (double)x[2], (double)x[3]));
+}
+
+__device__ __forceinline__ bool lc_total(const hals_sync& sy, const lane_ctl* ctl, int c, int ngran, int lane, double& total) {
+    const unsigned tag = hals_tag(sy, c);
+    const hals_word* base = hals_row(sy, c, ngran);
+    hals_word g0[LC_NP], g1[LC_NP];
+    unsigned spins = 0;
+    __builtin_amdgcn_s_sleep(32);
+    for (;;) {
+#pragma unroll
+        for (int i = 0; i < LC_NP; ++i) {
+            const int t = 256 * (i >> 2) + 4 * lane + (i & 3);
+            const int b = t < ngran ? t : 0;
+            g0[i] = __hip_atomic_load(base + 2 * (size_t)b, __ATOMIC_RELAXED, __HIP_MEMORY_SCOPE_AGENT);
+            g1[i] = __hip_atomic_load(base + 2 * (size_t)b + 1, __ATOMIC_RELAXED, __HIP_MEMORY_SCOPE_AGENT);
+        }
+        bool fresh = true;
+#pragma unroll
+        for (int i = 0; i < LC_NP; ++i) fresh = fresh && (unsigned)(g0[i] >> 32) == tag && (unsigned)(g1[i] >> 32) == tag;
+        if (__ballot(!fresh) == 0ull) break;
+        __builtin_amdgcn_s_sleep(16);
+        if (++spins > HALS_SPIN_LIMIT || ((spins & 63u) == 0u && __hip_atomic_load(&ctl->fin, __ATOMIC_RELAXED, LC_WG) != 0u)) return false;
+    }
+    double x[4];
+#pragma unroll
+    for (int j = 0; j < 4; ++j) {
+        double v = 0.0;
+        v += (4 * lane + j < ngran) ? hals_granule_value(g0[j], g1[j]) : 0.0;
+        v += (256 + 4 * lane + j < ngran) ? hals_granule_value(g0[j + 4], g1[j + 4]) : 0.0;
+        x[j] = v;
+    }
+    total = lc_rows_in_order(lc_sum4x64(x[0], x[1], x[2], x[3]));
+    return true;
+}
+
+__device__ __forceinline__ void lc_verdict(lane_ctl* ctl, int c, unsigned flag, int lane) {
+    if (lane == 0)
+        __hip_atomic_store(&ctl->ver[c & (LC_RING - 1)], ((unsigned long long)(unsigned)c << 32) | (unsigned long long)flag,
+                           __ATOMIC_RELAXED, LC_WG);
+}
+
+__device__ __forceinline__ void lc_comm_loop(const hals_args& a, lane_ctl* ctl, const float* nd, int ngran, int lane, double eps0, double eps) {
+    int done = 0;
+    bool ok = true;
+    for (int c = 1; c <= a.max_sweeps; ++c) {
+        if (!lc_wait_tags(ctl, c, lane)) { ok = false; lc_verdict(ctl, c, 2u, lane); break; }
+#pragma unroll
+        for (int h = 0; h < 2; ++h) {
+            const int gi = 2 * (int)blockIdx.x + h;
+            if (gi < ngran) {
+                const double bs = lc_half_sum(nd + (c & 1) * LC_COLS + 256 * h, lane);
+                if (lane == 0) lc_publish(a.sy, c, ngran, gi, bs);
+            }
+        }
+        double tot;
+        if (!lc_total(a.sy, ctl, c, ngran, lane, tot)) { ok = false; lc_verdict(ctl, c, 2u, lane); break; }
+        if (c == 1 && a.sweep0 == 0) eps0 = tot;
+        eps = tot;
+        done = c;
+        const bool on = hals_goes_on(eps, a.delta, eps0);
+        lc_verdict(ctl, c, on ? 0u : 1u, lane);
+        if (!on) break;
+    }
+    if (blockIdx.x == 0 && lane == 0) hals_status_finish(a.status, a.max_sweeps >= 1, a.sweep0, done, eps, eps0, !ok);
+}
+
+template <int RP>
+__global__ __launch_bounds__(LC_THREADS) void nnf_hals_comm_kernel(hals_args a, int ngran) {
+    static_assert(RP > 32 && RP <= 52, "the row-split ranks");
+    extern __shared__ __attribute__((aligned(16))) float lc_lds[];
+    float* b_lds = lc_lds;
+    float* nd_lds = lc_lds + (size_t)RP * LC_COLS;
+    lane_ctl* ctl = reinterpret_cast<lane_ctl*>(nd_lds + 2 * LC_COLS);
+    const int tid = threadIdx.x, lane = tid & 63, w = __builtin_amdgcn_readfirstlane(tid >> 6);
+    double eps0 = 0.0, eps = 1.0;
+    if (a.sweep0 > 0 && !hals_take_over(a.status, a.sweep0, a.delta, eps0, eps)) return;
+    for (int e = tid; e < (int)(sizeof(lane_ctl) / 4); e += LC_THREADS) reinterpret_cast<unsigned*>(ctl)[e] = 0u;
+    __syncthreads();
+    if (w == LC_CW) {
+        lc_comm_loop(a, ctl, nd_lds, ngran, lane, eps0, eps);
+        return;
+    }
+
+    const int64_t gtid = (int64_t)blockIdx.x * LC_COLS + tid;
+    const rsrc_t rv = __builtin_amdgcn_make_buffer_rsrc(a.V, 0, (int)(((int64_t)(a.r - 1) * a.ldv + a.ncols) * 4), 0x00020000);
+    const rsrc_t rb = __builtin_amdgcn_make_buffer_rsrc(const_cast<float*>(a.UtM), 0,
+                                                        (int)(((int64_t)(a.r - 1) * a.ldm + a.ncols) * 4), 0x00020000);
+    const rsrc_t rvs = __builtin_amdgcn_make_buffer_rsrc(const_cast<float*>(a.Vsrc), 0,
+                                                         (int)(((int64_t)(a.r - 1) * a.ldvs + a.ncols) * 4), 0x00020000);
+    const int ldv4 = (int)(a.ldv * 4), ldm4 = (int)(a.ldm * 4), ldvs4 = (int)(a.ldvs * 4);
+    const int voff0 = gtid < a.ncols ? (int)(gtid * 4) : (int)0x7ffffff0;
+    const bool all_live = a.dinv[2 * RP] != 0.f;
+    f32x2 v2[RP / 2], vb[RP / 2];
+    bool plain;
+    {
+        float b[RP];
+#pragma unroll
+        for (int k = 0; k < RP; ++k) {
+            v2[k / 2][k & 1] = __builtin_bit_cast(float, __builtin_amdgcn_raw_buffer_load_b32(rvs, voff0, k * ldvs4, 0));
+            b[k] = __builtin_bit_cast(float, __builtin_amdgcn_raw_buffer_load_b32(rb, voff0, k * ldm4, 0)) - a.sp;
+            b[k] *= a.dinv[2 * k];
+        }
+        float c = a.Gs[lane < RP ? lane * 64 + 63 : 63];
+#pragma unroll
+        for (int k = 0; k < RP; ++k) {
+            c = fmaf(v2[k / 2][k & 1], 0.f, c);
+            c = fmaf(b[k], 0.f, c);
+            asm volatile("" : "+v"(c));
+            b_lds[k * LC_COLS + tid] = b[k];
+        }
+        plain = all_live && __ballot(!(c == 0.f)) == 0ull;
+    }
+    asm volatile("s_waitcnt lgkmcnt(0)" ::: "memory");
+    const unsigned ba = (unsigned)(uintptr_t)(__attribute__((address_space(3))) float*)(b_lds + tid);
+    const hals_b_lds bsrc{ba, ba + 32u * LC_COLS * 4u, {0.f, 0.f}};
+
+    bool ok = true, stopped = false;
+    for (int s = 1; s <= a.max_sweeps; ++s) {
+#pragma unroll
+        for (int k = 0; k < RP / 2; ++k) vb[k] = v2[k];
+        const float f = plain ? hals_sweep_column_xy<RP, false>(v2, bsrc, a.Gs, a.dinv, hals_mid_none{})
+                              : hals_sweep_column_xy<RP, true>(v2, bsrc, a.Gs, a.dinv, hals_mid_none{});
+        nd_lds[(s & 1) * LC_COLS + tid] = gtid < a.ncols ? f : 0.f;
+        if (lane == 0) __hip_atomic_store(&ctl->tag[s & (LC_RING - 1)][w], (unsigned)s, __ATOMIC_RELEASE, LC_WG);
+        if (s >= 2) {
+            const unsigned long long* vp = &ctl->ver[(s - 1) & (LC_RING - 1)];
+            unsigned long long x = __hip_atomic_load(vp, __ATOMIC_RELAXED, LC_WG);
+            unsigned spins = 0;
+            while ((unsigned)(x >> 32) != (unsigned)(s - 1)) {
+                if (++spins > HALS_SPIN_LIMIT) { x = 2ull; break; }
+                if (spins < 64u) __builtin_amdgcn_s_sleep(1);
+                else __builtin_amdgcn_s_sleep(16);
+                x = __hip_atomic_load(vp, __ATOMIC_RELAXED, LC_WG);
+            }
+            const unsigned flag = (unsigned)__builtin_amdgcn_readfirstlane((int)(unsigned)x);
+            if (flag == 1u) { stopped = true; break; }
+            if (flag != 0u) { ok = false; break; }
+        }
+    }
+    if (!ok && lane == 0) __hip_atomic_store(&ctl->fin, 1u, __ATOMIC_RELAXED, LC_WG);
+    if (stopped || !ok) {
+#pragma unroll
+        for (int k = 0; k < RP / 2; ++k) v2[k] = vb[k];
+    }
+#pragma unroll
+    for (int k = 0; k < RP; ++k) {
+        const float val = v2[k / 2][k & 1];
+        __builtin_amdgcn_raw_buffer_store_b32(__builtin_bit_cast(unsigned, val), rv, voff0, k * ldv4, 0);
+    }
+    if (!ok && blockIdx.x == 0 && tid == 0) hals_status_finish(a.status, false, 0, 0, 0.0, 0.0, true);
+}
+
+template <int RP>
+static int comm_per_cu() {
+    static int cached = -1;
+    if (cached < 0) {
+        (void)hipFuncSetAttribute(reinterpret_cast<const void*>(&nnf_hals_comm_kernel<RP>), hipFuncAttributeMaxDynamicSharedMemorySize,
+                                  (int)lc_lds_bytes(RP));
+        int nb = 0;
+        const hipError_t e = hipOccupancyMaxActiveBlocksPerMultiprocessor(&nb, nnf_hals_comm_kernel<RP>, LC_THREADS, lc_lds_bytes(RP));
+        cached = hals_per_cu(e, nb, 1);
+    }
+    return cached;
+}
+template <int RP>
+static int comm_launch(const hals_args& a, int nblocks, hipStream_t st) {
+    if (comm_per_cu<RP>() < 1) return NNF_ERR_LAUNCH;
+    const int ngran = (int)nnf_cdiv(a.ncols, 256);
+    if (ngran > 64 * LC_NP || nblocks != (int)nnf_cdiv(a.ncols, LC_COLS) || a.mode != 0) return NNF_ERR_UNSUPPORTED;
+    hipLaunchKernelGGL((nnf_hals_comm_kernel<RP>), dim3(nblocks), dim3(LC_THREADS), lc_lds_bytes(RP), st, a, ngran);
+    NNF_CHECK_LAUNCH();
+    return NNF_OK;
+}
+
+#define LC_RANKS(X) X(40) X(48) X(50) X(52)
+int nnf_hals_comm_per_cu(int RP) {
+#define LC_PER_CU(v) case v: return comm_per_cu<v>();
+    switch (RP) { LC_RANKS(LC_PER_CU) default: return 0; }
+}
+int nnf_hals_comm_launch(int RP, const hals_args& a, int nblocks, hipStream_t st) {
+#define LC_LAUNCH(v) case v: return comm_launch<v>(a, nblocks, st);
+    switch (RP) { LC_RANKS(LC_LAUNCH) default: return NNF_ERR_UNSUPPORTED; }
+}
diff --git a/nn_fac_amd/csrc/k_hals_common.h b/nn_fac_amd/csrc/k_hals_common.h
--- a/nn_fac_amd/csrc/k_hals_common.h
+++ b/nn_fac_amd/csrc/k_hals_common.h
@@ -356,6 +356,9 @@
 int nnf_hals_fast_per_cu(int RP, bool resident);
 int nnf_hals_fast_launch(int RP, bool resident, const hals_args& a, int nblocks, hipStream_t);
 
+int nnf_hals_comm_per_cu(int RP);
+int nnf_hals_comm_launch(int RP, const hals_args& a, int nblocks, hipStream_t);
+
 int nnf_hals_wave_per_cu(int r, int cpw, int nw);
 int nnf_hals_wave_prep(const float* UtU, const float* UtU2, int64_t ldg, int r, float* Gw, unsigned* counter, double* status,
                        hipStream_t);
diff --git a/nn_fac_amd/csrc/k_hals_fast.hip b/nn_fac_amd/csrc/k_hals_fast.hip
--- a/nn_fac_amd/csrc/k_hals_fast.hip
+++ b/nn_fac_amd/csrc/k_hals_fast.hip
@@ -1,4 +1,5 @@
 #include "k_hals_common.h"
+#include "k_hals_lane_sweep.h"
 #include "k_parts.h"
 
 #ifndef HALS_PART
@@ -7,9 +8,6 @@
 #define NNF_PART HALS_PART
 
 NNF_BUILD_FLAGS(NNF_CAT(k_hals_fast, HALS_PART), "HALS_LATE_ISSUE=" NNF_STR(HALS_LATE_ISSUE) " HALS_MID_AT(R)=" NNF_STR(HALS_MID_AT(R)) " HALS_DBG=" NNF_STR(HALS_DBG))
-
-typedef float f32x16 __attribute__((ext_vector_type(16)));
-typedef float f32x8 __attribute__((ext_vector_type(8)));
 
 #define NNF_SLOAD2(d0, d1, base, off) \
     asm volatile("s_load_dwordx16 %0, %2, %3\n\ts_load_dwordx16 %1, %2, %4" : "=&s"(d0), "=&s"(d1) : "s"(base), "i"((off) * 4), "i"((off) * 4 + 64))
@@ -18,113 +16,6 @@
                  : "=&s"(d0), "=&s"(d1), "=&s"(dd) : "s"(base), "i"((off) * 4), "i"((off) * 4 + 64), "i"((doff) * 4))
 #define NNF_SWAIT2(d0, d1) asm volatile("s_waitcnt lgkmcnt(0)" : "+s"(d0), "+s"(d1))
 #define NNF_SWAIT3(d0, d1, dd) asm volatile("s_waitcnt lgkmcnt(0)" : "+s"(d0), "+s"(d1), "+s"(dd))
-
-template <int W>
-struct sgbuf {
-    f32x16 a, b;
-    f32x8 q;
-    f32x4 r;
-};
-template <int W, bool TIED>
-__device__ __forceinline__ void sg_issue(sgbuf<W>& d, uint64_t base, int off) {
-    constexpr int N16 = W / 16, N8 = (W % 16) / 8, N4 = (W % 8) / 4;
-    static_assert(W % 4 == 0 && N16 <= 2, "piece decomposition");
-    if constexpr (TIED) {
-        if constexpr (N16 >= 1) asm volatile("s_load_dwordx16 %0, %1, %2" : "+s"(d.a) : "s"(base), "i"(off * 4));
-        if constexpr (N16 >= 2) asm volatile("s_load_dwordx16 %0, %1, %2" : "+s"(d.b) : "s"(base), "i"(off * 4 + 64));
-        if constexpr (N8 == 1) asm volatile("s_load_dwordx8 %0, %1, %2" : "+s"(d.q) : "s"(base), "i"(off * 4 + 64 * N16));
-        if constexpr (N4 == 1) asm volatile("s_load_dwordx4 %0, %1, %2" : "+s"(d.r) : "s"(base), "i"(off * 4 + 64 * N16 + 32 * N8));
-    } else {
-        if constexpr (N16 >= 1) asm volatile("s_load_dwordx16 %0, %1, %2" : "=s"(d.a) : "s"(base), "i"(off * 4));
-        if constexpr (N16 >= 2) asm volatile("s_load_dwordx16 %0, %1, %2" : "=s"(d.b) : "s"(base), "i"(off * 4 + 64));
-        if constexpr (N8 == 1) asm volatile("s_load_dwordx8 %0, %1, %2" : "=s"(d.q) : "s"(base), "i"(off * 4 + 64 * N16));
-        if constexpr (N4 == 1) asm volatile("s_load_dwordx4 %0, %1, %2" : "=s"(d.r) : "s"(base), "i"(off * 4 + 64 * N16 + 32 * N8));
-    }
-}
-template <int W>
-__device__ __forceinline__ void sg_arrived(sgbuf<W>& d) {
-    constexpr int N16 = W / 16, N8 = (W % 16) / 8, N4 = (W % 8) / 4;
-    if constexpr (N16 >= 1) asm volatile("" : "+s"(d.a));
-    if constexpr (N16 >= 2) asm volatile("" : "+s"(d.b));
-    if constexpr (N8 == 1) asm volatile("" : "+s"(d.q));
-    if constexpr (N4 == 1) asm volatile("" : "+s"(d.r));
-}
-template <int W>
-__device__ __forceinline__ f32x2 sg_pair(const sgbuf<W>& d, int p) {
-    constexpr int N16 = W / 16, N8 = (W % 16) / 8;
-    const int j = 2 * p;
-    if (N16 >= 1 && j < 16) return f32x2{d.a[j], d.a[j + 1]};
-    if (N16 >= 2 && j < 32) return f32x2{d.b[j - 16], d.b[j - 15]};
-    const int j2 = j - 16 * N16;
-    if (N8 == 1 && j2 < 8) return f32x2{d.q[j2], d.q[j2 + 1]};
-    const int j3 = j2 - 8 * N8;
-    return f32x2{d.r[j3], d.r[j3 + 1]};
-}
-
-template <int R, bool GUARD, class MID>
-__device__ __forceinline__ float hals_sweep_column_xy(f32x2 (&v2)[R / 2], const float (&b)[R], const float* __restrict__ Gs,
-                                                      const float* __restrict__ nzp, const MID& mid) {
-    constexpr int RS = 64, P = R / 2, YW = 24, XW = (R - YW + 3) & ~3, XP = XW / 2;
-    static_assert(YW == 24, "the Y issue statement below is written for x16 + x8");
-    static_assert(R > 32 && R <= 64 && R % 2 == 0 && XW + YW <= RS && XW >= 8, "row split");
-    const uint64_t base = (uint64_t)Gs, nzb = (uint64_t)nzp;
-    sgbuf<XW> X;
-    sgbuf<YW> Y[2];
-    f32x2 dv[2];
-    float nd = 0.f;
-    sg_issue<XW, false>(X, base, 0);
-    sg_issue<YW, false>(Y[0], base, XW);
-    if constexpr (GUARD) asm volatile("s_load_dwordx2 %0, %1, %2" : "=s"(dv[0]) : "s"(nzb), "i"(0));
-#pragma unroll
-    for (int k = 0; k < R; ++k) {
-        const int cur = k & 1, nxt = cur ^ 1;
-        if (k == HALS_MID_AT(R)) mid();
-        if constexpr (GUARD) asm volatile("s_waitcnt lgkmcnt(0)" : "+s"(dv[cur]));
-        else asm volatile("s_waitcnt lgkmcnt(0)" ::: "memory");
-        sg_arrived<XW>(X);
-        sg_arrived<YW>(Y[cur]);
-        if (k + 1 < R) {
-            if constexpr (GUARD)
-                asm volatile("s_load_dwordx16 %0, %3, %4\n\ts_load_dwordx8 %1, %3, %5\n\ts_load_dwordx2 %2, %6, %7"
-                             : "=&s"(Y[nxt].a), "=&s"(Y[nxt].q), "=&s"(dv[nxt])
-                             : "s"(base), "i"(((k + 1) * RS + XW) * 4), "i"(((k + 1) * RS + XW + 16) * 4), "s"(nzb),
-                               "i"(8 * (k + 1)));
-            else
-                asm volatile("s_load_dwordx16 %0, %2, %3\n\ts_load_dwordx8 %1, %2, %4"
-                             : "=&s"(Y[nxt].a), "=&s"(Y[nxt].q)
-                             : "s"(base), "i"(((k + 1) * RS + XW) * 4), "i"(((k + 1) * RS + XW + 16) * 4));
-        }
-        f32x2 a0 = {0.f, 0.f}, a1 = {0.f, 0.f};
-#pragma unroll
-        for (int p = 0; p < XP; ++p) {
-            const f32x2 g = sg_pair<XW>(X, p);
-            if (p & 1) a1 = __builtin_elementwise_fma(g, v2[p], a1);
-            else a0 = __builtin_elementwise_fma(g, v2[p], a0);
-        }
-        asm volatile("" : "+v"(a0), "+v"(a1));
-        if (k + 1 < R) sg_issue<XW, true>(X, base, (k + 1) * RS);
-#pragma unroll
-        for (int p = XP; p < P; ++p) {
-            const f32x2 g = sg_pair<YW>(Y[cur], p - XP);
-            if (p & 1) a1 = __builtin_elementwise_fma(g, v2[p], a1);
-            else a0 = __builtin_elementwise_fma(g, v2[p], a0);
-        }
-        const f32x2 a = a0 + a1;
-        const float vk = v2[k / 2][k & 1];
-        const float x = b[k] - (a[0] + a[1]);
-        float dl;
-        if constexpr (GUARD) {
-            const float sel = !(x < -vk) ? x : -vk;
-            asm("v_mul_legacy_f32 %0, %1, %2" : "=v"(dl) : "s"(dv[cur][1]), "v"(sel));
-        } else {
-            asm("v_max_f32 %0, %1, -%2" : "=v"(dl) : "v"(x), "v"(vk));
-        }
-        v2[k / 2][k & 1] = vk + dl;
-        nd = fmaf(dl, dl, nd);
-        asm volatile("" : "+v"(nd));
-    }
-    return nd;
-}
 
 template <int R, bool KEEPB, class MID>
 __device__ __forceinline__ float hals_sweep_column(f32x2 (&v2)[R / 2], const float (&b)[KEEPB ? R : 1], rsrc_t rb, int voff,
@@ -222,7 +113,8 @@
     bool plain = false;
     auto sweep = [&](int voff, const auto& mid) -> float {
         if constexpr (XY) {
-            return plain ? hals_sweep_column_xy<RP, false>(v2, b, a.Gs, a.dinv, mid) : hals_sweep_column_xy<RP, true>(v2, b, a.Gs, a.dinv, mid);
+            return plain ? hals_sweep_column_xy<RP, false>(v2, hals_b_regs<RP>{b}, a.Gs, a.dinv, mid)
+                         : hals_sweep_column_xy<RP, true>(v2, hals_b_regs<RP>{b}, a.Gs, a.dinv, mid);
         } else {
             return hals_sweep_column<RP, KEEPB>(v2, b, rb, voff, ldm4, a.Gp, a.sp, mid);
         }
@@ -305,13 +197,14 @@
         bool merged = false;
         double tot_m = 0.0;
         if constexpr (RES && SPEC) {
-            if (a.mode == 0 && s >= 2 && !(HALS_DBG & 6)) {
+            if (a.mode == 0 && s >= 2 && !(HALS_DBG & 14)) {
                 ok = hals_sum_collect1<256>(a.sy, nd, bs, s - 1, nblocks, tot_m, red2[s & 1][0], red2[s & 1][1], &lds_flag, pf);
                 merged = true;
             }
         }
         if (!merged) {
-            if constexpr (RES) bs = hals_block_sum1<256>(nd, red2[s & 1][0]);
+            if constexpr (RES && (HALS_DBG & 8) != 0) bs = nd;
+            else if constexpr (RES) bs = hals_block_sum1<256>(nd, red2[s & 1][0]);
             else bs = nnf_block_sum_f64(nd, red);
         }
         if (a.mode == 1) {
@@ -327,9 +220,9 @@
             done = s;
             continue;
         }
-        if (!(HALS_DBG & 4)) hals_publish(a.sy, s, nblocks, bs);
+        if (!(HALS_DBG & 12)) hals_publish(a.sy, s, nblocks, bs);
         const int c = SPEC ? s - 1 : s;
-        if (c >= 1 && !(HALS_DBG & 6)) {
+        if (c >= 1 && !(HALS_DBG & 14)) {
             double tot;
             if (merged) tot = tot_m;
             else if constexpr (RES) ok = hals_collect1(a.sy, c, nblocks, tot, red2[s & 1][1], &lds_flag, pf);
diff --git a/nn_fac_amd/csrc/k_hals_lane_sweep.h b/nn_fac_amd/csrc/k_hals_lane_sweep.h
--- /dev/null
+++ b/nn_fac_amd/csrc/k_hals_lane_sweep.h
@@ -0,0 +1,135 @@
+#pragma once
+#include "k_hals_common.h"
+
+typedef float f32x16 __attribute__((ext_vector_type(16)));
+typedef float f32x8 __attribute__((ext_vector_type(8)));
+
+template <int W>
+struct sgbuf {
+    f32x16 a, b;
+    f32x8 q;
+    f32x4 r;
+};
+template <int W, bool TIED>
+__device__ __forceinline__ void sg_issue(sgbuf<W>& d, uint64_t base, int off) {
+    constexpr int N16 = W / 16, N8 = (W % 16) / 8, N4 = (W % 8) / 4;
+    static_assert(W % 4 == 0 && N16 <= 2, "piece decomposition");
+    if constexpr (TIED) {
+        if constexpr (N16 >= 1) asm volatile("s_load_dwordx16 %0, %1, %2" : "+s"(d.a) : "s"(base), "i"(off * 4));
+        if constexpr (N16 >= 2) asm volatile("s_load_dwordx16 %0, %1, %2" : "+s"(d.b) : "s"(base), "i"(off * 4 + 64));
+        if constexpr (N8 == 1) asm volatile("s_load_dwordx8 %0, %1, %2" : "+s"(d.q) : "s"(base), "i"(off * 4 + 64 * N16));
+        if constexpr (N4 == 1) asm volatile("s_load_dwordx4 %0, %1, %2" : "+s"(d.r) : "s"(base), "i"(off * 4 + 64 * N16 + 32 * N8));
+    } else {
+        if constexpr (N16 >= 1) asm volatile("s_load_dwordx16 %0, %1, %2" : "=s"(d.a) : "s"(base), "i"(off * 4));
+        if constexpr (N16 >= 2) asm volatile("s_load_dwordx16 %0, %1, %2" : "=s"(d.b) : "s"(base), "i"(off * 4 + 64));
+        if constexpr (N8 == 1) asm volatile("s_load_dwordx8 %0, %1, %2" : "=s"(d.q) : "s"(base), "i"(off * 4 + 64 * N16));
+        if constexpr (N4 == 1) asm volatile("s_load_dwordx4 %0, %1, %2" : "=s"(d.r) : "s"(base), "i"(off * 4 + 64 * N16 + 32 * N8));
+    }
+}
+template <int W>
+__device__ __forceinline__ void sg_arrived(sgbuf<W>& d) {
+    constexpr int N16 = W / 16, N8 = (W % 16) / 8, N4 = (W % 8) / 4;
+    if constexpr (N16 >= 1) asm volatile("" : "+s"(d.a));
+    if constexpr (N16 >= 2) asm volatile("" : "+s"(d.b));
+    if constexpr (N8 == 1) asm volatile("" : "+s"(d.q));
+    if constexpr (N4 == 1) asm volatile("" : "+s"(d.r));
+}
+template <int W>
+__device__ __forceinline__ f32x2 sg_pair(const sgbuf<W>& d, int p) {
+    constexpr int N16 = W / 16, N8 = (W % 16) / 8;
+    const int j = 2 * p;
+    if (N16 >= 1 && j < 16) return f32x2{d.a[j], d.a[j + 1]};
+    if (N16 >= 2 && j < 32) return f32x2{d.b[j - 16], d.b[j - 15]};
+    const int j2 = j - 16 * N16;
+    if (N8 == 1 && j2 < 8) return f32x2{d.q[j2], d.q[j2 + 1]};
+    const int j3 = j2 - 8 * N8;
+    return f32x2{d.r[j3], d.r[j3 + 1]};
+}
+
+template <int R>
+struct hals_b_regs {
+    const float (&b)[R];
+    __device__ __forceinline__ void issue(int) {}
+    __device__ __forceinline__ float get(int k) { return b[k]; }
+};
+constexpr int HALS_B_PITCH = 512;
+struct hals_b_lds {
+    unsigned a0, a1;
+    float v[2];
+    __device__ __forceinline__ void issue(int k) {
+        if (k < 32) asm volatile("ds_read_b32 %0, %1 offset:%2" : "=v"(v[k & 1]) : "v"(a0), "i"(k * HALS_B_PITCH * 4));
+        else asm volatile("ds_read_b32 %0, %1 offset:%2" : "=v"(v[k & 1]) : "v"(a1), "i"((k - 32) * HALS_B_PITCH * 4));
+    }
+    __device__ __forceinline__ float get(int k) {
+        asm volatile("" : "+v"(v[k & 1]));
+        return v[k & 1];
+    }
+};
+
+template <int R, bool GUARD, class MID, class BSRC>
+__device__ __forceinline__ float hals_sweep_column_xy(f32x2 (&v2)[R / 2], BSRC b, const float* __restrict__ Gs,
+                                                      const float* __restrict__ nzp, const MID& mid) {
+    constexpr int RS = 64, P = R / 2, YW = 24, XW = (R - YW + 3) & ~3, XP = XW / 2;
+    static_assert(YW == 24, "the Y issue statement below is written for x16 + x8");
+    static_assert(R > 32 && R <= 64 && R % 2 == 0 && XW + YW <= RS && XW >= 8, "row split");
+    const uint64_t base = (uint64_t)Gs, nzb = (uint64_t)nzp;
+    sgbuf<XW> X;
+    sgbuf<YW> Y[2];
+    f32x2 dv[2];
+    float nd = 0.f;
+    sg_issue<XW, false>(X, base, 0);
+    sg_issue<YW, false>(Y[0], base, XW);
+    if constexpr (GUARD) asm volatile("s_load_dwordx2 %0, %1, %2" : "=s"(dv[0]) : "s"(nzb), "i"(0));
+    b.issue(0);
+#pragma unroll
+    for (int k = 0; k < R; ++k) {
+        const int cur = k & 1, nxt = cur ^ 1;
+        if (k == HALS_MID_AT(R)) mid();
+        if constexpr (GUARD) asm volatile("s_waitcnt lgkmcnt(0)" : "+s"(dv[cur]));
+        else asm volatile("s_waitcnt lgkmcnt(0)" ::: "memory");
+        sg_arrived<XW>(X);
+        sg_arrived<YW>(Y[cur]);
+        const float bk = b.get(k);
+        if (k + 1 < R) {
+            if constexpr (GUARD)
+                asm volatile("s_load_dwordx16 %0, %3, %4\n\ts_load_dwordx8 %1, %3, %5\n\ts_load_dwordx2 %2, %6, %7"
+                             : "=&s"(Y[nxt].a), "=&s"(Y[nxt].q), "=&s"(dv[nxt])
+                             : "s"(base), "i"(((k + 1) * RS + XW) * 4), "i"(((k + 1) * RS + XW + 16) * 4), "s"(nzb),
+                               "i"(8 * (k + 1)));
+            else
+                asm volatile("s_load_dwordx16 %0, %2, %3\n\ts_load_dwordx8 %1, %2, %4"
+                             : "=&s"(Y[nxt].a), "=&s"(Y[nxt].q)
+                             : "s"(base), "i"(((k + 1) * RS + XW) * 4), "i"(((k + 1) * RS + XW + 16) * 4));
+            b.issue(k + 1);
+        }
+        f32x2 a0 = {0.f, 0.f}, a1 = {0.f, 0.f};
+#pragma unroll
+        for (int p = 0; p < XP; ++p) {
+            const f32x2 g = sg_pair<XW>(X, p);
+            if (p & 1) a1 = __builtin_elementwise_fma(g, v2[p], a1);
+            else a0 = __builtin_elementwise_fma(g, v2[p], a0);
+        }
+        asm volatile("" : "+v"(a0), "+v"(a1));
+        if (k + 1 < R) sg_issue<XW, true>(X, base, (k + 1) * RS);
+#pragma unroll
+        for (int p = XP; p < P; ++p) {
+            const f32x2 g = sg_pair<YW>(Y[cur], p - XP);
+            if (p & 1) a1 = __builtin_elementwise_fma(g, v2[p], a1);
+            else a0 = __builtin_elementwise_fma(g, v2[p], a0);
+        }
+        const f32x2 a = a0 + a1;
+        const float vk = v2[k / 2][k & 1];
+        const float x = bk - (a[0] + a[1]);
+        float dl;
+        if constexpr (GUARD) {
+            const float sel = !(x < -vk) ? x : -vk;
+            asm("v_mul_legacy_f32 %0, %1, %2" : "=v"(dl) : "s"(dv[cur][1]), "v"(sel));
+        } else {
+            asm("v_max_f32 %0, %1, -%2" : "=v"(dl) : "v"(x), "v"(vk));
+        }
+        v2[k / 2][k & 1] = vk + dl;
+        nd = fmaf(dl, dl, nd);
+        asm volatile("" : "+v"(nd));
+    }
+    return nd;
+}
diff --git a/nn_fac_amd/csrc/k_hals_plan.h b/nn_fac_amd/csrc/k_hals_plan.h
--- a/nn_fac_amd/csrc/k_hals_plan.h
+++ b/nn_fac_amd/csrc/k_hals_plan.h
@@ -28,6 +28,7 @@
     size_t lds = 0;
     bool hadamard = false, copy = false, prep = true;
     bool gs = false;
+    bool comm = false;
     size_t gram_floats = 0, mfma_floats = 0, snap_floats = 0;
 };
 
@@ -37,6 +38,7 @@
     int (*lane)(int RP, bool resident);
     int (*mfma)(int RP);
     int (*generic)(int mode, hals_layout layout, int r, size_t lds_bytes, int cap);
+    int (*lane_comm)(int RP);
 };
 
 static inline int pick_rp(int r) {
@@ -96,6 +98,8 @@
 constexpr size_t HALS_GENERIC_LDS_MAX = (size_t)150 * 1024;
 constexpr size_t HALS_GENERIC_SHM_FIXED = 16 + 3 * 2 * 8 + 64;
 
+constexpr int HALS_COMM_MAX_GRANULES = 512;
+
 static inline int64_t hals_cap(int cus, int per_cu) {
     const int64_t c = (int64_t)per_cu * cus;
     return c < NNF_HALS_MAX_BLOCKS ? c : NNF_HALS_MAX_BLOCKS;
@@ -116,12 +120,12 @@
     const bool sweeps = q.nsweeps > 0;
     const char force = q.force;
     p.RP = pick_rp(r);
-    const bool mfma = !generic && sweeps && force != 'l' && force != 'q' && force != 'w' && nnf_hals_mfma_supported(p.RP) &&
+    const bool mfma = !generic && sweeps && force != 'l' && force != 'c' && force != 'q' && force != 'w' && nnf_hals_mfma_supported(p.RP) &&
                       (force == 'm' || (p.RP >= 64 && n > 32768));
     const bool pin_mfma = force == 'm' && mfma;
 
     const bool wave_shape = !generic && q.mode == 0 && q.sweep0 == 0;
-    if (wave_shape && force != 'l' && force != 'q' && !pin_mfma) {
+    if (wave_shape && force != 'l' && force != 'c' && force != 'q' && !pin_mfma) {
         for (int cpw = 1; cpw <= 2; ++cpw) {
             int nw = 0;
             const int need = nnf_hals_wave_grid(n, cpw, &nw);
@@ -141,7 +145,7 @@
     if (force == 'w' && wave_shape) return hals_refuse(p, NNF_ERR_UNSUPPORTED);
 
     auto quad_32bit = [&](int64_t ld) { return (int64_t)(r + 16) * ld * 4 < (int64_t)0x7fff0000; };
-    if (!generic && force != 'l' && !pin_mfma && (n <= 32768 || force == 'q') && quad_32bit(q.ldv > q.ldm ? q.ldv : q.ldm)) {
+    if (!generic && force != 'l' && force != 'c' && !pin_mfma && (n <= 32768 || force == 'q') && quad_32bit(q.ldv > q.ldm ? q.ldv : q.ldm)) {
         const int ch = (r + 3) / 4, pc = occ.quad(ch);
         const int64_t need = nnf_cdiv(n, 16);
         if (pc > 0 && need <= hals_cap(cus, pc)) {
@@ -200,6 +204,11 @@
     if (lane_pc < 1) return hals_refuse(p, NNF_ERR_LAUNCH);
     if (lane_fits) {
         p.layout = HL_LANE_RES, p.nblocks = (int)need, p.per_cu = lane_pc;
+        if (q.mode == 0 && p.gs && need <= HALS_COMM_MAX_GRANULES && force != 'l' && (force == 'c' || need > cus)) {
+            const int pc = occ.lane_comm ? occ.lane_comm(p.RP) : 0;
+            const int64_t need2 = nnf_cdiv(n, 512);
+            if (pc > 0 && need2 <= hals_cap(cus, pc)) p.comm = true, p.nblocks = (int)need2, p.per_cu = pc;
+        }
         return p;
     }
     if (q.snapshots) return hals_refuse(p, NNF_ERR_UNSUPPORTED);
@@ -211,9 +220,9 @@
 
 static inline void hals_report(FILE* f, const hals_shape& q, const hals_plan& p, const char* more = "") {
     fprintf(f, "[nnf hals] r=%d ncols=%lld mode=%d sweeps=%d sweep0=%d flags=%u -> %s grid=%d per_cu=%d cpw=%d nw=%d ch=%d "
-            "RP=%d gs=%d lds=%zu hadamard=%d copy=%d prep=%d err=%d%s\n", q.r, (long long)q.ncols, q.mode, q.nsweeps, q.sweep0,
+            "RP=%d gs=%d lds=%zu hadamard=%d copy=%d prep=%d err=%d comm=%d%s\n", q.r, (long long)q.ncols, q.mode, q.nsweeps, q.sweep0,
             q.flags, hals_layout_name[p.layout], p.nblocks, p.per_cu, p.cpw, p.nw, p.ch, p.RP, p.gs, p.lds, p.hadamard, p.copy,
-            p.prep, p.err, more);
+            p.prep, p.err, p.comm, more);
 }
 
 static inline int64_t hals_resident_columns(int cus, const hals_occupancy& occ, int r) {
```
